# laclouis5/StructureDetector

Measured on AMD Instinct MI355X. Metric: images/sec (train fwd+bwd) and decode us/img at 512x512, higher is better.
Workload: dtype f32

## Files before the change

### include/sdnet_hip.h

```cpp
#ifndef SDNET_HIP_H
#define SDNET_HIP_H

#include <stddef.h>
#include <stdint.h>

#ifdef __cplusplus
extern "C" {
#endif

#define SD_ERR_INVALID   (-1)
#define SD_ERR_WORKSPACE (-2)
#define SD_ERR_ALIGN     (-3)

#define SD_MAX_TOPK 1024

typedef void* sd_stream_t;

int         sd_version(void);
const char* sd_last_error(void);
int         sd_build_flags(void);


int sd_clamped_sigmoid(const float* x, float* y, int64_t n, sd_stream_t stream);

// ... 218 lines not shown
int sd_conv2d_fwd_bf16(const void* x_nhwc_bf16, const void* w_krsc_bf16, void* y_nhwc_bf16, const sd_conv_desc* d,
                       const float* scale, const float* shift, const void* residual_bf16, int res_up2, int relu,
                       void* workspace, size_t workspace_bytes, sd_stream_t stream);
int sd_maxpool3x3s2_fwd_bf16(const void* x_bf16, void* y_bf16, int B, int Hi, int Wi, int C, sd_stream_t stream);
int sd_stem_bn_relu_maxpool_fwd_bf16(const float* x_nchw, const float* w, const float* scale, const float* shift, void* y_bf16,
                                     const sd_conv_desc* d, sd_stream_t stream);

int sd_cast_bf16_to_f32(const void* x_bf16, float* y, int64_t n, sd_stream_t stream);
size_t sd_conv2d_fwd_bf16_bn_stats_workspace_bytes(const sd_conv_desc* d);
int sd_conv2d_fwd_bf16_bn_stats(const void* x_nhwc_bf16, const void* w_krsc_bf16, void* y_nhwc_bf16, const sd_conv_desc* d, float eps,
                                float momentum, float* running_mean, float* running_var, float* mean, float* invstd,
                                void* workspace, size_t workspace_bytes, sd_stream_t stream);
int sd_conv2d_stem_fwd_bn_stats_bf16mm(const float* x_nchw, const float* w, float* y, const sd_conv_desc* d, float eps, float momentum,
                                       float* running_mean, float* running_var, float* mean, float* invstd,
                                       void* workspace, size_t workspace_bytes, sd_stream_t stream);
int sd_conv2d_stem_fwd_bn_stats_bf16(const float* x_nchw, const float* w, void* y_bf16, const sd_conv_desc* d, float eps, float momentum,
                                     float* running_mean, float* running_var, float* mean, float* invstd, void* workspace,
                                     size_t workspace_bytes, sd_stream_t stream);
int sd_bn_relu_maxpool_fwd_bf16(const void* x_bf16, int B, int Hi, int Wi, int C, const float* mean, const float* invstd, const float* gamma,
                                const float* beta, void* y_pool_bf16, uint8_t* idx, sd_stream_t stream);
int sd_maxpool_bn_relu_bwd_bf16(const void* dpool_bf16, const uint8_t* idx, const void* x_bf16, int B, int Hi, int Wi, int C, const float* mean,
                                const float* invstd, const float* gamma, const float* beta, float* dx, float* dgamma, float* dbeta, int accumulate,
                                void* workspace, size_t workspace_bytes, sd_stream_t stream);
int sd_maxpool_bn_relu_bwd_bf16_dx16(const void* dpool_bf16, const uint8_t* idx, const void* x_bf16, int B, int Hi, int Wi, int C, const float* mean,
                                     const float* invstd, const float* gamma, const float* beta, void* dx_bf16, float* dgamma, float* dbeta,
                                     int accumulate, void* workspace, size_t workspace_bytes, sd_stream_t stream);
int sd_conv2d_transpose_weights_bf16(const float* w, void* w_t_bf16, int Cout, int taps, int Cin, sd_stream_t stream);

int sd_conv2d_fwd_bf16_head_supported(const sd_conv_desc* d, int head_co);
size_t sd_head_split_bf16_bytes(void);
int sd_head_split_bf16(const float* head_w, const float* head_bias, int head_co, void* prepared, sd_stream_t stream);
int sd_conv2d_fwd_bf16_head(const void* x_bf16, const void* w_bf16, const sd_conv_desc* d, const float* scale, const float* shift, int relu,
                            const void* head_prepared, int head_co, float* head_y, sd_stream_t stream);
int sd_conv2d_dgrad_bf16(const void* dy_bf16, const void* w_t_bf16, void* dx_bf16, const sd_conv_desc* d, const void* residual_bf16,
                         int res_mode, sd_stream_t stream);
size_t sd_conv2d_wgrad_bf16_workspace_bytes(const sd_conv_desc* d);
int sd_conv2d_wgrad_bf16(const void* dy_bf16, const void* x_nhwc_bf16, float* dw_krsc, const sd_conv_desc* d, int accumulate,
                         void* workspace, size_t workspace_bytes, sd_stream_t stream);
int sd_bn_apply_bf16(const void* x, void* y, int64_t M, int C, const float* mean, const float* invstd, const float* gamma,
                     const float* beta, const void* residual, int relu, uint8_t* relu_mask_out, sd_stream_t stream);
int sd_bn_bwd_bf16(const void* dy, const void* x, const void* y, int relu, int64_t M, int C, const float* mean, const float* invstd,
                   const float* gamma, const float* beta, void* dx, void* g_out, float* dgamma, float* dbeta, int accumulate,
                   void* workspace, size_t workspace_bytes, sd_stream_t stream);
int sd_bn_train_stats_bf16(const void* x, int64_t M, int C, float eps, float momentum, float* running_mean, float* running_var,
                           float* mean, float* invstd, void* workspace, size_t workspace_bytes, sd_stream_t stream);
int sd_col_sum_bf16(const void* x, int64_t M, int C, float* out, int accumulate, void* workspace, size_t workspace_bytes, sd_stream_t stream);
int sd_upsample2x_bwd_bf16(const void* dy, const void* add, void* dx, int B, int H, int W, int C, sd_stream_t stream);
int sd_head_fwd_bf16(const void* x_nhwc_bf16, const float* w, const float* bias, float* y_nchw, int B, int HW, int C,
                     int Co, sd_stream_t stream);
int sd_conv2d_dgrad(const float* dy_nhwc, const float* w_t, float* dx_nhwc, const sd_conv_desc* d,
                    const float* residual, sd_stream_t stream);
int sd_conv2d_dgrad_half_res(const float* dy, const float* w_t, float* dx, const sd_conv_desc* d, const float* residual_half,
                             sd_stream_t stream);
int sd_conv2d_transpose_weights(const float* w, float* w_t, int Cout, int taps, int Cin, sd_stream_t stream);
int sd_conv2d_transpose_weights_batched(const float* w_base, void* w_t_base, const int* table, int nconv, int total_blocks, int out_bf16,
                                        sd_stream_t stream);
size_t sd_conv2d_wgrad_workspace_bytes(const sd_conv_desc* d);
int sd_conv2d_wgrad(const float* dy_nhwc, const float* x_nhwc, float* dw_krsc, const sd_conv_desc* d,
                    int accumulate, void* workspace, size_t workspace_bytes, sd_stream_t stream);
size_t sd_conv2d_stem_wgrad_workspace_bytes(const sd_conv_desc* d);
int sd_conv2d_stem_wgrad(const float* dy_nhwc, const float* x_nchw, float* dw_krsc, const sd_conv_desc* d,
                         int accumulate, void* workspace, size_t workspace_bytes, sd_stream_t stream);
int sd_conv2d_stem_wgrad_bf16mm(const float* dy, const float* x_nchw, float* dw, const sd_conv_desc* d, int accumulate, void* workspace,
                                size_t workspace_bytes, sd_stream_t stream);
int sd_conv2d_stem_wgrad_bf16(const void* dy_bf16, const float* x_nchw, float* dw, const sd_conv_desc* d, int accumulate, void* workspace,
                              size_t workspace_bytes, sd_stream_t stream);

size_t sd_col_reduce_workspace_bytes(int64_t M, int C);
int sd_bn_train_stats(const float* x, int64_t M, int C, float eps, float momentum, float* running_mean,
                      float* running_var, float* mean, float* invstd, void* workspace, size_t workspace_bytes,
                      sd_stream_t stream);
int sd_bn_apply(const float* x, float* y, int64_t M, int C, const float* mean, const float* invstd,
                const float* gamma, const float* beta, const float* residual, int relu, uint8_t* relu_mask_out,
                sd_stream_t stream);
int sd_bn_fold(const float* gamma, const float* beta, const float* running_mean, const float* running_var,
               float eps, int C, float* scale, float* shift, sd_stream_t stream);
int sd_bn_bwd(const float* dy, const float* x, const float* y, int relu, int64_t M, int C, const float* mean,
              const float* invstd, const float* gamma, const float* beta, float* dx, float* g_out, float* dgamma,
              float* dbeta, int accumulate, void* workspace, size_t workspace_bytes, sd_stream_t stream);
int sd_col_sum(const float* x, int64_t M, int C, float* out, int accumulate, void* workspace,
               size_t workspace_bytes, sd_stream_t stream);

int sd_maxpool3x3s2_fwd(const float* x, float* y, uint8_t* idx, int B, int Hi, int Wi, int C, sd_stream_t stream);
int sd_maxpool3x3s2_bwd(const float* dy, const uint8_t* idx, float* dx, int B, int Hi, int Wi, int C, sd_stream_t stream);
int sd_bn_relu_maxpool_fwd(const float* x, int B, int Hi, int Wi, int C, const float* mean, const float* invstd, const float* gamma,
                           const float* beta, float* y_pool, uint8_t* idx, sd_stream_t stream);
int sd_maxpool_bn_relu_bwd(const float* dpool, const uint8_t* idx, const float* x, int B, int Hi, int Wi, int C, const float* mean,
                           const float* invstd, const float* gamma, const float* beta, float* dx, float* dgamma, float* dbeta,
                           int accumulate, void* workspace, size_t workspace_bytes, sd_stream_t stream);
int sd_upsample2x_bwd(const float* dy, const float* add, float* dx, int B, int H, int W, int C, sd_stream_t stream);

#define SD_HEAD_MAX_CO 256
int sd_head_fwd(const float* x_nhwc, const float* w, const float* bias, float* y_nchw, int B, int HW, int C, int Co,
                sd_stream_t stream);
size_t sd_head_bwd_workspace_bytes(int B, int HW, int C, int Co);
int sd_head_bwd(const float* dy_nchw, const float* x_nhwc, const float* w, float* dx_nhwc, float* dw, float* dbias,
                int B, int HW, int C, int Co, int accumulate, void* workspace, size_t workspace_bytes, sd_stream_t stream);
int sd_head_bwd_bf16(const float* dy, const void* x_bf16, const float* w, void* dx_bf16, float* dw, float* dbias, int B, int HW, int C, int Co,
                     int accumulate, void* workspace, size_t workspace_bytes, sd_stream_t stream);

int sd_adam_step(float* param, const float* grad, float* exp_avg, float* exp_avg_sq, int64_t n, int step,
                 float lr, float beta1, float beta2, float eps, float grad_scale, sd_stream_t stream);

#define SD_OPTIM_STATUS_BYTES 16
size_t sd_grad_sumsq_workspace_bytes(int64_t n);
int sd_grad_sumsq(const float* grad, int64_t n, void* workspace, size_t workspace_bytes, sd_stream_t stream);
int sd_optim_step(float* param, const float* grad, float* exp_avg, float* exp_avg_sq, int64_t n, int step,
                  float lr, float beta1, float beta2, float eps, float grad_scale, float weight_decay,
                  const uint8_t* decay_mask, float max_norm, const void* partials, int npartials, float* ema,
                  float ema_decay, void* status, sd_stream_t stream);

#define SD_COMM_ID_BYTES 128
int sd_allreduce_unique_id(void* id_out);
int sd_allreduce_init(const void* id, int rank, int world, void** comm_out);
int sd_allreduce_run(void* comm, float* buf, int64_t count, sd_stream_t stream);
int sd_allreduce_destroy(void* comm);

int sd_comm_sim_copy(const void* src, void* dst, size_t src_bytes, size_t move_bytes, int workgroups, float gbps, sd_stream_t stream);

double sd_mfma_bf16_stream_flops(int iters);
int    sd_mfma_bf16_stream(const void* operands64k, float* out, int iters, sd_stream_t stream);

int sd_bn_stats_from_sums(const double* sums, int C, float eps, float momentum, float* running_mean, float* running_var, float* mean,
                          float* invstd, sd_stream_t stream);
int sd_bn_bwd_means_from_sums(const double* sums, int C, float* means_out, sd_stream_t stream);
int sd_bn_stats_sums(const float* partial, int rows, int64_t M, int C, double* sums, float* scratch, sd_stream_t stream);
int sd_bn_bwd_sums(const float* partial, int rows, int64_t M, int C, float* dgamma, float* dbeta, int accumulate, double* sums,
                   float* scratch, sd_stream_t stream);
int sd_bn_train_sums(const float* x, int64_t M, int C, double* sums, void* workspace, size_t workspace_bytes, sd_stream_t stream);
int sd_bn_train_sums_bf16(const void* x, int64_t M, int C, double* sums, void* workspace, size_t workspace_bytes, sd_stream_t stream);
int sd_conv2d_fwd_bn_stats_rows(const sd_conv_desc* d, int bf16);
int sd_conv2d_fwd_bn_sums(const float* x, const float* w, float* y, const sd_conv_desc* d, double* sums, void* workspace,
// ... 47 lines not shown
```

### structuredetector_amd/_lib.py

```python
from __future__ import annotations

import ctypes as C
import os
from pathlib import Path

import torch

_HERE = Path(__file__).resolve().parent
LIB_PATH = Path(os.environ.get("SDNET_HIP_LIB", _HERE / "csrc" / "libsdnet_hip.so"))

_lib = None

c_f32p = C.c_void_p
c_i64 = C.c_int64
c_int = C.c_int
c_float = C.c_float
c_size = C.c_size_t
c_vp = C.c_void_p


class SdError(RuntimeError):
    pass


# ... 64 lines not shown
    "sd_preprocess_images_list_jitter": (c_int, [c_vp] + [c_int] * 5 + [c_vp, c_vp, c_int, c_vp, c_vp, c_int, c_vp, c_vp, c_vp, C.POINTER(c_float),
                                                            C.POINTER(c_float), c_vp, c_vp, c_size, c_vp]),
    "sd_preprocess_affine_workspace_bytes": (c_size, [c_int] * 5),
    "sd_preprocess_images_affine": (c_int, [c_vp] + [c_int] * 5 + [c_vp, c_vp, c_int, c_vp, c_vp, c_int, c_vp, c_vp, c_vp, c_vp, C.POINTER(C.c_ubyte),
                                            C.POINTER(c_float), C.POINTER(c_float), c_vp, c_vp, c_size, c_vp]),
    "sd_preprocess_images_list_affine": (c_int, [c_vp] + [c_int] * 5 + [c_vp, c_vp, c_int, c_vp, c_vp, c_int, c_vp, c_vp, c_vp, c_vp, C.POINTER(C.c_ubyte),
                                                 C.POINTER(c_float), C.POINTER(c_float), c_vp, c_vp, c_size, c_vp]),
    "sd_preprocess_mosaic_workspace_bytes": (c_size, [c_int] * 5),
    "sd_preprocess_images_mosaic": (c_int, [c_vp] + [c_int] * 5 + [c_vp, c_vp, c_int, c_vp, c_vp, c_int, c_vp, c_vp, c_vp, c_vp, c_vp, c_vp,
                                            C.POINTER(C.c_ubyte), C.POINTER(c_float), C.POINTER(c_float), c_vp, c_vp, c_size, c_vp]),
    "sd_preprocess_images_list_mosaic": (c_int, [c_vp] + [c_int] * 5 + [c_vp, c_vp, c_int, c_vp, c_vp, c_int, c_vp, c_vp, c_vp, c_vp, c_vp, c_vp,
                                                 C.POINTER(C.c_ubyte), C.POINTER(c_float), C.POINTER(c_float), c_vp, c_vp, c_size, c_vp]),
    "sd_preprocess_window_workspace_bytes": (c_size, [c_int] * 4),
    "sd_preprocess_images_window": (c_int, [c_vp] + [c_int] * 7 + [c_vp, c_vp, c_int, c_vp, c_vp, c_int, c_vp, c_int, c_int] + [c_vp] * 6 +
                                    [C.POINTER(C.c_ubyte), C.POINTER(c_float), C.POINTER(c_float), c_vp, c_vp, c_size, c_vp]),
    "sd_preprocess_images_list_window": (c_int, [c_vp] + [c_int] * 7 + [c_vp, c_vp, c_int, c_vp, c_vp, c_int, c_vp, c_int, c_int] + [c_vp] * 6 +
                                         [C.POINTER(C.c_ubyte), C.POINTER(c_float), C.POINTER(c_float), c_vp, c_vp, c_size, c_vp]),
    "sd_render_targets": (c_int, [c_vp, c_vp, c_vp, c_int, c_int, c_int, c_int, c_float, c_vp, c_vp]),
    "sd_loss_workspace_bytes": (c_size, [c_int] * 5),
    "sd_loss_fwd": (c_int, [C.POINTER(LossDesc), c_vp, c_vp, c_size, c_vp]),
    "sd_loss_fwd_per_image": (c_int, [C.POINTER(LossDesc), c_vp, c_vp, c_size, c_vp]),
    "sd_loss_bwd": (c_int, [C.POINTER(LossDesc), c_vp, c_vp, c_vp, c_vp]),
    "sd_conv2d_fwd_workspace_bytes": (c_size, [C.POINTER(ConvDesc)]),
    "sd_conv2d_fwd": (c_int, [c_vp, c_vp, c_vp, C.POINTER(ConvDesc), c_vp, c_vp, c_vp, c_int, c_int, c_vp, c_size, c_vp]),
    "sd_conv2d_fwd_sb_supported": (c_int, [C.POINTER(ConvDesc), c_int]),
    "sd_conv2d_fwd_sb_workspace_bytes": (c_size, [C.POINTER(ConvDesc), c_int]),
    "sd_conv2d_fwd_sb_state_bytes": (c_size, [C.POINTER(ConvDesc), c_int]),
    "sd_conv2d_fwd_sb": (c_int, [c_vp, c_vp, c_vp, C.POINTER(ConvDesc), c_vp, c_vp, c_vp, c_int, c_int, c_int, c_vp, c_size, c_vp, c_size, c_vp]),
    "sd_conv2d_stem_fwd_workspace_bytes": (c_size, [C.POINTER(ConvDesc)]),
    "sd_conv2d_stem_fwd": (c_int, [c_vp, c_vp, c_vp, C.POINTER(ConvDesc), c_vp, c_vp, c_int, c_int, c_vp, c_size, c_vp]),
    "sd_cast_f32_to_bf16": (c_int, [c_vp, c_vp, c_i64, c_vp]),
    "sd_conv2d_fwd_bf16_workspace_bytes": (c_size, [C.POINTER(ConvDesc)]),
    "sd_conv2d_fwd_bf16": (c_int, [c_vp, c_vp, c_vp, C.POINTER(ConvDesc), c_vp, c_vp, c_vp, c_int, c_int, c_vp, c_size, c_vp]),
    "sd_conv2d_fwd_bf16_head_supported": (c_int, [C.POINTER(ConvDesc), c_int]),
    "sd_head_split_bf16_bytes": (c_size, []),
    "sd_head_split_bf16": (c_int, [c_vp, c_vp, c_int, c_vp, c_vp]),
    "sd_conv2d_fwd_bf16_head": (c_int, [c_vp, c_vp, C.POINTER(ConvDesc), c_vp, c_vp, c_int, c_vp, c_int, c_vp, c_vp]),
    "sd_cast_bf16_to_f32": (c_int, [c_vp, c_vp, c_i64, c_vp]),
    "sd_conv2d_fwd_bf16_bn_stats_workspace_bytes": (c_size, [c_vp]),
    "sd_conv2d_fwd_bf16_bn_stats": (c_int, [c_vp, c_vp, c_vp, c_vp, c_float, c_float, c_vp, c_vp, c_vp, c_vp, c_vp, c_size, c_vp]),
    "sd_conv2d_wgrad_bf16_workspace_bytes": (c_size, [c_vp]),
    "sd_conv2d_wgrad_bf16": (c_int, [c_vp, c_vp, c_vp, c_vp, c_int, c_vp, c_size, c_vp]),
    "sd_conv2d_transpose_weights_bf16": (c_int, [c_vp, c_vp, c_int, c_int, c_int, c_vp]),
    "sd_conv2d_dgrad_bf16": (c_int, [c_vp, c_vp, c_vp, c_vp, c_vp, c_int, c_vp]),
    "sd_bn_apply_bf16": (c_int, [c_vp, c_vp, c_i64, c_int, c_vp, c_vp, c_vp, c_vp, c_vp, c_int, c_vp, c_vp]),
    "sd_bn_bwd_bf16": (c_int, [c_vp, c_vp, c_vp, c_int, c_i64, c_int, c_vp, c_vp, c_vp, c_vp, c_vp, c_vp, c_vp, c_vp, c_int, c_vp, c_size, c_vp]),
    "sd_bn_train_stats_bf16": (c_int, [c_vp, c_i64, c_int, c_float, c_float, c_vp, c_vp, c_vp, c_vp, c_vp, c_size, c_vp]),
    "sd_col_sum_bf16": (c_int, [c_vp, c_i64, c_int, c_vp, c_int, c_vp, c_size, c_vp]),
    "sd_upsample2x_bwd_bf16": (c_int, [c_vp, c_vp, c_vp, c_int, c_int, c_int, c_int, c_vp]),
    "sd_maxpool3x3s2_fwd_bf16": (c_int, [c_vp, c_vp, c_int, c_int, c_int, c_int, c_vp]),
    "sd_stem_bn_relu_maxpool_fwd_bf16": (c_int, [c_vp, c_vp, c_vp, c_vp, c_vp, c_vp, c_vp]),
    "sd_head_fwd_bf16": (c_int, [c_vp, c_vp, c_vp, c_vp, c_int, c_int, c_int, c_int, c_vp]),
    "sd_conv2d_dgrad": (c_int, [c_vp, c_vp, c_vp, C.POINTER(ConvDesc), c_vp, c_vp]),
    "sd_conv2d_transpose_weights": (c_int, [c_vp, c_vp, c_int, c_int, c_int, c_vp]),
    "sd_conv2d_transpose_weights_batched": (c_int, [c_vp, c_vp, c_vp, c_int, c_int, c_int, c_vp]),
    "sd_conv2d_wgrad_workspace_bytes": (c_size, [C.POINTER(ConvDesc)]),
    "sd_conv2d_wgrad": (c_int, [c_vp, c_vp, c_vp, C.POINTER(ConvDesc), c_int, c_vp, c_size, c_vp]),
    "sd_conv2d_stem_wgrad_workspace_bytes": (c_size, [C.POINTER(ConvDesc)]),
    "sd_conv2d_stem_wgrad": (c_int, [c_vp, c_vp, c_vp, C.POINTER(ConvDesc), c_int, c_vp, c_size, c_vp]),
    "sd_conv2d_stem_wgrad_bf16mm": (c_int, [c_vp, c_vp, c_vp, C.POINTER(ConvDesc), c_int, c_vp, c_size, c_vp]),
    "sd_conv2d_stem_wgrad_bf16": (c_int, [c_vp, c_vp, c_vp, C.POINTER(ConvDesc), c_int, c_vp, c_size, c_vp]),
    "sd_col_reduce_workspace_bytes": (c_size, [c_i64, c_int]),
    "sd_bn_train_stats": (c_int, [c_vp, c_i64, c_int, c_float, c_float, c_vp, c_vp, c_vp, c_vp, c_vp, c_size, c_vp]),
    "sd_bn_apply": (c_int, [c_vp, c_vp, c_i64, c_int, c_vp, c_vp, c_vp, c_vp, c_vp, c_int, c_vp, c_vp]),
    "sd_bn_fold": (c_int, [c_vp, c_vp, c_vp, c_vp, c_float, c_int, c_vp, c_vp, c_vp]),
    "sd_bn_bwd": (c_int, [c_vp, c_vp, c_vp, c_int, c_i64, c_int, c_vp, c_vp, c_vp, c_vp, c_vp, c_vp, c_vp, c_vp, c_int, c_vp, c_size, c_vp]),
    "sd_col_sum": (c_int, [c_vp, c_i64, c_int, c_vp, c_int, c_vp, c_size, c_vp]),
    "sd_maxpool3x3s2_fwd": (c_int, [c_vp, c_vp, c_vp, c_int, c_int, c_int, c_int, c_vp]),
    "sd_maxpool3x3s2_bwd": (c_int, [c_vp, c_vp, c_vp, c_int, c_int, c_int, c_int, c_vp]),
    "sd_upsample2x_bwd": (c_int, [c_vp, c_vp, c_vp, c_int, c_int, c_int, c_int, c_vp]),
    "sd_head_fwd": (c_int, [c_vp, c_vp, c_vp, c_vp, c_int, c_int, c_int, c_int, c_vp]),
    "sd_head_bwd_workspace_bytes": (c_size, [c_int] * 4),
    "sd_head_bwd": (c_int, [c_vp] * 6 + [c_int] * 5 + [c_vp, c_size, c_vp]),
    "sd_head_bwd_bf16": (c_int, [c_vp] * 6 + [c_int] * 5 + [c_vp, c_size, c_vp]),
    "sd_adam_step": (c_int, [c_vp, c_vp, c_vp, c_vp, c_i64, c_int, c_float, c_float, c_float, c_float, c_float, c_vp]),
    "sd_grad_sumsq_workspace_bytes": (c_size, [c_i64]),
    "sd_grad_sumsq": (c_int, [c_vp, c_i64, c_vp, c_size, c_vp]),
    "sd_optim_step": (c_int, [c_vp, c_vp, c_vp, c_vp, c_i64, c_int, c_float, c_float, c_float, c_float, c_float, c_float, c_vp, c_float, c_vp, c_int,
                              c_vp, c_float, c_vp, c_vp]),
    "sd_conv2d_kernel_name": (C.c_char_p, [c_vp, c_int]),
    "sd_set_option": (c_int, [C.c_char_p, c_int]),
    "sd_decode_set_option": (c_int, [C.c_char_p, c_int]),
    "sd_decode_kernel_names": (C.c_char_p, [c_int] * 9),
    "sd_conv2d_stem_fwd_bn_stats_workspace_bytes": (c_size, [c_vp]),
    "sd_conv2d_stem_fwd_bn_stats": (c_int, [c_vp, c_vp, c_vp, c_vp, c_float, c_float, c_vp, c_vp, c_vp, c_vp, c_vp, c_size, c_vp]),
    "sd_conv2d_stem_fwd_bn_stats_bf16mm": (c_int, [c_vp, c_vp, c_vp, c_vp, c_float, c_float, c_vp, c_vp, c_vp, c_vp, c_vp, c_size, c_vp]),
    "sd_conv2d_stem_fwd_bn_stats_bf16": (c_int, [c_vp, c_vp, c_vp, c_vp, c_float, c_float, c_vp, c_vp, c_vp, c_vp, c_vp, c_size, c_vp]),
    "sd_conv2d_dgrad_half_res": (c_int, [c_vp] * 6),
    "sd_bn_relu_maxpool_fwd": (c_int, [c_vp, c_int, c_int, c_int, c_int] + [c_vp] * 7),
    "sd_bn_relu_maxpool_fwd_bf16": (c_int, [c_vp, c_int, c_int, c_int, c_int] + [c_vp] * 7),
    "sd_maxpool_bn_relu_bwd": (c_int, [c_vp, c_vp, c_vp, c_int, c_int, c_int, c_int] + [c_vp] * 7 + [c_int, c_vp, c_size, c_vp]),
    "sd_maxpool_bn_relu_bwd_bf16": (c_int, [c_vp, c_vp, c_vp, c_int, c_int, c_int, c_int] + [c_vp] * 7 + [c_int, c_vp, c_size, c_vp]),
    "sd_maxpool_bn_relu_bwd_bf16_dx16": (c_int, [c_vp, c_vp, c_vp, c_int, c_int, c_int, c_int] + [c_vp] * 7 + [c_int, c_vp, c_size, c_vp]),
    "sd_conv2d_fwd_bn_stats_workspace_bytes": (c_size, [c_vp]),
    "sd_conv2d_fwd_bn_stats": (c_int, [c_vp, c_vp, c_vp, c_vp, c_float, c_float, c_vp, c_vp, c_vp, c_vp, c_vp, c_size, c_vp]),
    "sd_conv2d_dgrad_bn_reduce_workspace_bytes": (c_size, [c_vp]),
    "sd_conv2d_dgrad_bn_reduce": (c_int, [c_vp] * 5 + [c_vp, c_vp, c_int] + [c_vp] * 6 + [c_int, c_vp, c_vp, c_size, c_vp]),
    "sd_bn_bwd_finalize": (c_int, [c_vp, c_int, c_i64, c_int, c_vp, c_vp, c_int, c_vp, c_vp, c_vp]),
    "sd_bn_bwd_apply": (c_int, [c_vp, c_vp, c_vp, c_int, c_i64, c_int] + [c_vp] * 8),
    "sd_bn_finalize_scratch_rows": (c_int, [c_int]),
    "sd_bn_finalize_stats": (c_int, [c_vp, c_int, c_i64, c_int, c_float, c_float, c_vp, c_vp, c_vp, c_vp, c_vp, c_vp]),
    "sd_bn_stats_from_sums": (c_int, [c_vp, c_int, c_float, c_float, c_vp, c_vp, c_vp, c_vp, c_vp]),
    "sd_bn_bwd_means_from_sums": (c_int, [c_vp, c_int, c_vp, c_vp]),
    "sd_bn_stats_sums": (c_int, [c_vp, c_int, c_i64, c_int, c_vp, c_vp, c_vp]),
    "sd_bn_bwd_sums": (c_int, [c_vp, c_int, c_i64, c_int, c_vp, c_vp, c_int, c_vp, c_vp, c_vp]),
    "sd_bn_train_sums": (c_int, [c_vp, c_i64, c_int, c_vp, c_vp, c_size, c_vp]),
# ... 114 lines not shown
```

### structuredetector_amd/csrc/sd_conv.hip

```cpp
#include <string.h>
#include "sd_common.h"
#include "sd_mfma.h"
#include "sd_conv_rows.h"

#ifndef SD_S2_LPT
#define SD_S2_LPT 1
#endif
namespace sd {


#ifndef SD_IGEMM_DMA
#define SD_IGEMM_DMA 1
#endif
#ifndef SD_ABLATE_HOT
#define SD_ABLATE_HOT 0
#endif
#ifndef SD_ABLATE_STORE
#define SD_ABLATE_STORE 0
#endif
#ifndef SD_ABLATE_PATCH
#define SD_ABLATE_PATCH 0
#endif
#if SD_ABLATE_HOT || SD_ABLATE_STORE || SD_ABLATE_PATCH || defined(SD_PP_ABL) || defined(SD_RS_ABL)
#warning "timing-only ablation build: this libsdnet_hip.so computes WRONG RESULTS; the Python loader refuses it unless SDNET_ALLOW_ABLATION=1"
// ... 10 lines not shown
#if defined(SD_PP_ABL) || defined(SD_RS_ABL) || defined(SD_SB_ABL) || defined(SD_SHAPE_EXP) || defined(SD_W16_ABL) || defined(SD_SR_ABL) || defined(SD_SF_ABL)
#define SD_EXPERIMENT_FLAG 16
#else
#define SD_EXPERIMENT_FLAG 0
#endif
void sd_nn_set_pool_pair(int v);
extern "C" int sd_build_flags(void) { return (SD_ABLATE_HOT ? 1 : 0) | (SD_ABLATE_STORE ? 2 : 0) | (SD_ABLATE_PATCH ? 4 : 0) | SD_TRACE_FLAG | SD_EXPERIMENT_FLAG; }

#ifndef SD_SHAPE_EXP
#define SD_SHAPE_EXP 0
#else
#define SD_SHAPE_EXP_BUILD 1
#endif
__device__ __forceinline__ f32x16 mfma_shape_exp(bf16x8 a, bf16x8 b, f32x16 c) {
    f32x4 c0 = __builtin_shufflevector(c, c, 0, 1, 2, 3), c1 = __builtin_shufflevector(c, c, 4, 5, 6, 7);
    c0 = __builtin_amdgcn_mfma_f32_16x16x32_bf16(a, b, c0, 0, 0, 0);
    c1 = __builtin_amdgcn_mfma_f32_16x16x32_bf16(b, a, c1, 0, 0, 0);
    c[0] = c0[0]; c[1] = c0[1]; c[2] = c0[2]; c[3] = c0[3]; c[4] = c1[0]; c[5] = c1[1]; c[6] = c1[2]; c[7] = c1[3];
    return c;
}
#define SD_MFMA_BF16(BIT, a, b, c) (((SD_SHAPE_EXP) & (BIT)) ? mfma_shape_exp(a, b, c) : __builtin_amdgcn_mfma_f32_32x32x16_bf16(a, b, c, 0, 0, 0))

#ifndef SD_IGEMM_LATE_DMA
#define SD_IGEMM_LATE_DMA 0
#endif
constexpr int NBUF = 2;
constexpr int BM = 128, BK = 32, LDK = BK;

struct ConvArgs {
    const void* x;
    const void* w;
    void* y;
    const float* scale;
    const float* shift;
    const void* res;
    int B, Hi, Wi, Ck, Ho, Wo, Nn, R, S;
    int mul, div, off, rsign;
    int relu, res_up2;
    int M, nk, kchunks;
    int splits;
    float* part;
    const float* bn_x;
    const float* bn_y;
    const float *bn_mean, *bn_invstd, *bn_gamma, *bn_beta;
    int bn_relu;
    float* stat;
    int pt_tw_log2, pt_pw, pt_pieces, pt_rolling, pt_flip;
    int pt_strip_log2;
    int par;
    const uint16_t* head_w;
    const float* head_b;
    float* head_y;
    int head_co;
};

__device__ __attribute__((aligned(128))) float g_zero_line[64];


__device__ __forceinline__ void s2_tile(int bid, int nwg, int n_tiles, int off, int& cls, int& tq, int& n_idx, int& tile_m) {
    if (SD_S2_LPT && (nwg & 31) == 0) {
        const int xcd = bid & 7, pos = bid >> 3, per = nwg >> 5;
        const int k4 = pos / per, within = xcd * per + (pos - k4 * per);
        cls = (off & 1) ? (k4 == 0 ? 3 : k4 == 3 ? 0 : k4) : k4;
        tq = within / n_tiles; n_idx = within - tq * n_tiles;
    } else {
        const int tile = xcd_remap(bid, nwg), tm = tile / n_tiles;
        cls = tm & 3; tq = tm >> 2; n_idx = tile - tm * n_tiles;
    }
    tile_m = 4 * tq + cls;
}


__device__ __forceinline__ float f4c(const float4& v, int t) { return t == 0 ? v.x : (t == 1 ? v.y : (t == 2 ? v.z : v.w)); }

struct BnRed4 { float4 mu, is, ga, be, s, q; };
__device__ __forceinline__ void bnred4_init(BnRed4& b, const ConvArgs& p, int n) {
    b.mu = *reinterpret_cast<const float4*>(p.bn_mean + n); b.is = *reinterpret_cast<const float4*>(p.bn_invstd + n);
    b.ga = b.be = b.s = b.q = make_float4(0.f, 0.f, 0.f, 0.f);
    if (p.bn_relu == 2) { b.ga = *reinterpret_cast<const float4*>(p.bn_gamma + n); b.be = *reinterpret_cast<const float4*>(p.bn_beta + n); }
}
__device__ __forceinline__ void bnred4_add(BnRed4& b, const ConvArgs& p, float4 g, int64_t m, int n) {
    const int64_t i = m * p.Nn + n;
    const float4 xv = *reinterpret_cast<const float4*>(p.bn_x + i);
    const float4 xh = make_float4((xv.x - b.mu.x) * b.is.x, (xv.y - b.mu.y) * b.is.y, (xv.z - b.mu.z) * b.is.z, (xv.w - b.mu.w) * b.is.w);
    if (p.bn_relu == 1) {
        const float4 yy = *reinterpret_cast<const float4*>(p.bn_y + i);
        g.x = yy.x > 0.f ? g.x : 0.f; g.y = yy.y > 0.f ? g.y : 0.f; g.z = yy.z > 0.f ? g.z : 0.f; g.w = yy.w > 0.f ? g.w : 0.f;
    } else if (p.bn_relu == 3) {
        const uint8_t mb = reinterpret_cast<const uint8_t*>(p.bn_y)[i >> 2];
        g.x = (mb & 1) ? g.x : 0.f; g.y = (mb & 2) ? g.y : 0.f; g.z = (mb & 4) ? g.z : 0.f; g.w = (mb & 8) ? g.w : 0.f;
    } else if (p.bn_relu == 2) {
        g.x = (xh.x * b.ga.x + b.be.x) > 0.f ? g.x : 0.f; g.y = (xh.y * b.ga.y + b.be.y) > 0.f ? g.y : 0.f;
        g.z = (xh.z * b.ga.z + b.be.z) > 0.f ? g.z : 0.f; g.w = (xh.w * b.ga.w + b.be.w) > 0.f ? g.w : 0.f;
    }
    b.s.x += g.x; b.s.y += g.y; b.s.z += g.z; b.s.w += g.w;
    b.q.x += g.x * xh.x; b.q.y += g.y * xh.y; b.q.z += g.z * xh.z; b.q.w += g.w * xh.w;
}
template <int LPR>
__device__ __forceinline__ void bnred4_wave_sum(BnRed4& b) {
#pragma unroll
    for (int o = LPR; o < 64; o <<= 1) {
        b.s.x += __shfl_xor(b.s.x, o); b.s.y += __shfl_xor(b.s.y, o); b.s.z += __shfl_xor(b.s.z, o); b.s.w += __shfl_xor(b.s.w, o);
        b.q.x += __shfl_xor(b.q.x, o); b.q.y += __shfl_xor(b.q.y, o); b.q.z += __shfl_xor(b.q.z, o); b.q.w += __shfl_xor(b.q.w, o);
    }
}

// ... 380 lines not shown
            if (BF16) {
                uint2 pk;
                pk.x = (uint32_t)f2bf(v.x) | ((uint32_t)f2bf(v.y) << 16);
                pk.y = (uint32_t)f2bf(v.z) | ((uint32_t)f2bf(v.w) << 16);
                *reinterpret_cast<uint2*>(reinterpret_cast<uint16_t*>(p.y) + (int64_t)m * p.Nn + n) = pk;
            } else {
                *reinterpret_cast<float4*>(reinterpret_cast<float*>(p.y) + (int64_t)m * p.Nn + n) = v;
                if (bwd_red) bnred4_add(br, p, v, m, n);
            }
        };
        if constexpr (BF16) {
#pragma unroll
            for (int it = 0; it < 64 / RPI; ++it) out_row(it, rr[it], nullptr);
        } else if (pre32) {
#pragma unroll
            for (int it = 0; it < 64 / RPI; ++it) out_row(it, make_uint2(0u, 0u), &rf[it]);
        } else {
#pragma unroll 4
            for (int it = 0; it < 64 / RPI; ++it) out_row(it, make_uint2(0u, 0u), nullptr);
        }
        if (bwd_red) {
            bnred4_wave_sum<LPR>(br);
            if ((wave >> 1) == 1 && lane < LPR) {
                *reinterpret_cast<float4*>(&statred[0][wn0 + c4]) = br.s; *reinterpret_cast<float4*>(&statred[1][wn0 + c4]) = br.q;
            }
            __syncthreads();
            if ((wave >> 1) == 0 && lane < LPR) {
                float* dst = p.stat + (int64_t)tile_m * 2 * p.Nn + n;
                const float4 a = *reinterpret_cast<const float4*>(&statred[0][wn0 + c4]), bq = *reinterpret_cast<const float4*>(&statred[1][wn0 + c4]);
                *reinterpret_cast<float4*>(dst) = make_float4(br.s.x + a.x, br.s.y + a.y, br.s.z + a.z, br.s.w + a.w);
                *reinterpret_cast<float4*>(dst + p.Nn) = make_float4(br.q.x + bq.x, br.q.y + bq.y, br.q.z + bq.z, br.q.w + bq.w);
            }
            red_done = true;
        }
    }
    if (fwd_stat || (bwd_red && !red_done)) {
#pragma unroll
        for (int ni = 0; ni < NT; ++ni) {
            sv[ni] += __shfl_xor(sv[ni], 32); qv[ni] += __shfl_xor(qv[ni], 32);
            if ((wave >> 1) == 1 && fh == 0) { statred[0][wn0 + ni * 32 + fr] = sv[ni]; statred[1][wn0 + ni * 32 + fr] = qv[ni]; }
        }
        __syncthreads();
        if ((wave >> 1) == 0 && fh == 0) {
            float* dst = p.stat + (int64_t)tile_m * 2 * p.Nn + n0;
#pragma unroll
            for (int ni = 0; ni < NT; ++ni) {
                const int c = wn0 + ni * 32 + fr;
                dst[c] = sv[ni] + statred[0][c]; dst[p.Nn + c] = qv[ni] + statred[1][c];
            }
        }
    }
}

template <int BN, int WM, int WN, int MT, int NTW, bool FWD, bool BF16 = false, bool VEC = false, typename RowMap, typename ResMap>
__device__ __forceinline__ void tile_epilogue(const ConvArgs& p, f32x16 (&acc)[MT][NTW], RowMap row_to_m, ResMap row_to_res, int tid, int wave, int fr,
                                              int fh, int wm0, int wn0, int n0, int tile_m, float* T0 = nullptr, float* T1 = nullptr) {
    const bool fwd_stat = FWD && p.stat && !p.bn_x;
    const bool bwd_red = !BF16 && p.stat && p.bn_x;
    float sv[NTW], qv[NTW];
#pragma unroll
    for (int ni = 0; ni < NTW; ++ni) {
        sv[ni] = qv[ni] = 0.f;
        if (fwd_stat) {
#pragma unroll
            for (int mi = 0; mi < MT; ++mi)
#pragma unroll
                for (int e = 0; e < 16; ++e) { const float a = BF16 ? bf2f(f2bf(acc[mi][ni][e])) : acc[mi][ni][e]; sv[ni] += a; qv[ni] += a * a; }
        }
    }
    const int lane = tid & 63;
    bool red_done = false;
    __shared__ float statred[2][BN];
    if (VEC && NTW == 2) {
        const int c4 = (lane & 15) * 4, n = n0 + wn0 + c4;
        float4 sc4 = make_float4(1.f, 1.f, 1.f, 1.f), sh4 = make_float4(0.f, 0.f, 0.f, 0.f);
        if (p.scale) sc4 = *reinterpret_cast<const float4*>(p.scale + n);
        if (p.shift) sh4 = *reinterpret_cast<const float4*>(p.shift + n);
        BnRed4 br;
        if (bwd_red) bnred4_init(br, p, n);
        const bool two = T1 != nullptr;
        const int npass = two ? MT / 2 : MT, rpp = two ? 64 : 32;
        for (int h = 0; h < npass; ++h) {
            uint2 rr[16] = {};
            if constexpr (BF16) {
                if (p.res) {
#pragma unroll
                    for (int it = 0; it < 16; ++it) {
                        if (it * 4 < rpp) {
                            const int trow = wm0 + h * rpp + it * 4 + (lane >> 4);
                            const int m = row_to_m(trow);
                            const int64_t rm = m < 0 ? -1 : (p.res_up2 ? (int64_t)row_to_res(trow, m) : (int64_t)m);
                            rr[it] = *reinterpret_cast<const uint2*>(reinterpret_cast<const uint16_t*>(p.res) + (rm >= 0 ? rm * p.Nn : 0) + n);
                        }
                    }
                }
            }
#pragma unroll
            for (int ni = 0; ni < NTW; ++ni)
#pragma unroll
                for (int e = 0; e < 16; ++e) {
                    const int r = (e & 3) + 8 * (e >> 2) + 4 * fh;
                    float v0 = 0.f, v1 = 0.f;
#pragma unroll
                    for (int mi = 0; mi < MT; ++mi) {
                        if (two ? mi == 2 * h : mi == h) v0 = acc[mi][ni][e];
                        if (two && mi == 2 * h + 1) v1 = acc[mi][ni][e];
                    }
                    T0[r * 64 + ni * 32 + fr] = v0;
                    if (two) T1[r * 64 + ni * 32 + fr] = v1;
                }
            auto out_row = [&](int it, uint2 r16) {
                const int rl = it * 4 + (lane >> 4);
                const int trow = wm0 + h * rpp + rl;
                const int m = row_to_m(trow);
                if (m < 0) return;
                float4 v = *reinterpret_cast<const float4*>((rl < 32 ? T0 : T1) + (rl & 31) * 64 + c4);
                v.x = v.x * sc4.x + sh4.x; v.y = v.y * sc4.y + sh4.y; v.z = v.z * sc4.z + sh4.z; v.w = v.w * sc4.w + sh4.w;
                if (p.res) {
                    const int64_t rm = p.res_up2 ? (int64_t)row_to_res(trow, m) : (int64_t)m;
                    if (rm >= 0) {
                        if (BF16) {
                            v.x += bf2f((uint16_t)(r16.x & 0xffff)); v.y += bf2f((uint16_t)(r16.x >> 16));
                            v.z += bf2f((uint16_t)(r16.y & 0xffff)); v.w += bf2f((uint16_t)(r16.y >> 16));
                        } else {
                            const float4 r = *reinterpret_cast<const float4*>(reinterpret_cast<const float*>(p.res) + rm * p.Nn + n);
                            v.x += r.x; v.y += r.y; v.z += r.z; v.w += r.w;
                        }
                    }
                }
                if (p.relu) { v.x = fmaxf(v.x, 0.f); v.y = fmaxf(v.y, 0.f); v.z = fmaxf(v.z, 0.f); v.w = fmaxf(v.w, 0.f); }
                if (BF16) {
                    uint2 pk;
                    pk.x = (uint32_t)f2bf(v.x) | ((uint32_t)f2bf(v.y) << 16);
                    pk.y = (uint32_t)f2bf(v.z) | ((uint32_t)f2bf(v.w) << 16);
                    *reinterpret_cast<uint2*>(reinterpret_cast<uint16_t*>(p.y) + (int64_t)m * p.Nn + n) = pk;
                } else {
                    *reinterpret_cast<float4*>(reinterpret_cast<float*>(p.y) + (int64_t)m * p.Nn + n) = v;
                    if (bwd_red) bnred4_add(br, p, v, m, n);
                }
            };
            if constexpr (BF16) {
#pragma unroll
                for (int it = 0; it < 16; ++it)
                    if (it * 4 < rpp) out_row(it, rr[it]);
            } else {
#pragma unroll 4
                for (int it = 0; it < 16; ++it) {
                    if (it * 4 >= rpp) break;
                    out_row(it, make_uint2(0u, 0u));
                }
            }
        }
        if (bwd_red) {
            bnred4_wave_sum<16>(br);
            if (tid < 2 * BN) statred[tid / BN][tid % BN] = 0.f;
            __syncthreads();
            for (int wr = 1; wr < WM; ++wr) {
                if (wave / WN == wr && lane < 16) {
                    float4* a = reinterpret_cast<float4*>(&statred[0][wn0 + c4]);
                    float4* bq = reinterpret_cast<float4*>(&statred[1][wn0 + c4]);
                    *a = make_float4(a->x + br.s.x, a->y + br.s.y, a->z + br.s.z, a->w + br.s.w);
                    *bq = make_float4(bq->x + br.q.x, bq->y + br.q.y, bq->z + br.q.z, bq->w + br.q.w);
                }
                __syncthreads();
            }
            if (wave / WN == 0 && lane < 16) {
                float* dst = p.stat + (int64_t)tile_m * 2 * p.Nn + n;
                const float4 a = *reinterpret_cast<const float4*>(&statred[0][wn0 + c4]), bq = *reinterpret_cast<const float4*>(&statred[1][wn0 + c4]);
                *reinterpret_cast<float4*>(dst) = make_float4(br.s.x + a.x, br.s.y + a.y, br.s.z + a.z, br.s.w + a.w);
                *reinterpret_cast<float4*>(dst + p.Nn) = make_float4(br.q.x + bq.x, br.q.y + bq.y, br.q.z + bq.z, br.q.w + bq.w);
            }
            red_done = true;
        }
    } else {
#pragma unroll
    for (int ni = 0; ni < NTW; ++ni) {
        const int n = n0 + wn0 + ni * 32 + fr;
        const float sc = p.scale ? p.scale[n] : 1.f;
        const float sh = p.shift ? p.shift[n] : 0.f;
        float bmu = 0.f, bis = 0.f, bga = 0.f, bbe = 0.f;
        if (bwd_red) {
            bmu = p.bn_mean[n]; bis = p.bn_invstd[n];
            if (p.bn_relu == 2) { bga = p.bn_gamma[n]; bbe = p.bn_beta[n]; }
        }
#pragma unroll
        for (int mi = 0; mi < MT; ++mi) {
#pragma unroll
            for (int e = 0; e < 16; ++e) {
                const int trow = wm0 + mi * 32 + (e & 3) + 8 * (e >> 2) + 4 * fh;
                const int m = row_to_m(trow);
                if (m < 0) continue;
                float v = acc[mi][ni][e] * sc + sh;
                if (p.res) {
                    const int64_t rm = p.res_up2 ? row_to_res(trow, m) : m;
                    const bool has = rm >= 0;
                    if (has) v += BF16 ? bf2f(reinterpret_cast<const uint16_t*>(p.res)[rm * p.Nn + n]) : reinterpret_cast<const float*>(p.res)[rm * p.Nn + n];
                }
                if (p.relu) v = fmaxf(v, 0.f);
                if (BF16) reinterpret_cast<uint16_t*>(p.y)[(int64_t)m * p.Nn + n] = f2bf(v);
                else if (!SD_ABLATE_STORE || v == 123.456f) reinterpret_cast<float*>(p.y)[(int64_t)m * p.Nn + n] = v;
                if (bwd_red) SD_BNRED_TERM(v, m, n, sv[ni], qv[ni])
            }
        }
// ... 393 lines not shown
        f32x4 a00 = lds_read128_async<0>(aa[0]), a01 = lds_read128_async<0>(aa[1]);                \
        f32x4 a02 = a00, a03 = a00;                                                                \
        if (MT == 4) { a02 = lds_read128_async<0>(aa[MT - 2]); a03 = lds_read128_async<0>(aa[MT - 1]); } \
        f32x4 b00 = lds_read128_async<0>(bb), b01 = lds_read128_async<TSTR>(bb);                   \
        f32x4 a10 = lds_read128_async<0>(aa[0] ^ 32u), a11 = lds_read128_async<0>(aa[1] ^ 32u);    \
        f32x4 a12 = a10, a13 = a10;                                                                \
        if (MT == 4) { a12 = lds_read128_async<0>(aa[MT - 2] ^ 32u); a13 = lds_read128_async<0>(aa[MT - 1] ^ 32u); } \
        f32x4 b10 = lds_read128_async<0>(bb ^ 32u), b11 = lds_read128_async<TSTR>(bb ^ 32u);       \
         \
        if (BF16 || SD_PATCH_READS_FIRST_F32) {                                                    \
            PT_ISSUE_B(cc + ((t) + 2) / 9, ((t) + 2) % 9, ((t) + 2) % 3)                               \
        if (rolling) {                                                                             \
             \
            if ((t) < 8) {                                                                         \
                const int row = (t) < 4 ? 2 + (t) / 2 : ((t) - 4) / 2;                             \
                const int cch = (t) < 4 ? cc : cc + 1;                                             \
                if (cch < nchunks) {                                                               \
                    if (((t) & 1) == 0) { PT_PATCH(3 * row, Pt, cch * KC) ++n_iss; }               \
                    else {                                                                         \
                        if (PT_OWN(3 * row + 1)) { PT_PATCH(3 * row + 1, Pt, cch * KC) ++n_iss; }  \
                        if (PT_OWN(3 * row + 2)) { PT_PATCH(3 * row + 2, Pt, cch * KC) ++n_iss; }  \
                    }                                                                              \
                }                                                                                  \
            }                                                                                      \
        } else if ((t) < 7 && cc + 1 < nchunks && PT_OWN(t)) {                                     \
            PT_PATCH(t, pt_nxt, (cc + 1) * KC) ++n_iss;                                            \
        }                                                                                          \
        }                                                                                          \
        if (MT == 4) { SD_LDS_WAIT6(6, a00, a01, a02, a03, b00, b01); } else { SD_LDS_WAIT4(4, a00, a01, b00, b01); } \
        PT_MFMA_GROUP(a00, a01, a02, a03, b00, b01)                                                \
        if (MT == 4) { SD_LDS_WAIT6(0, a10, a11, a12, a13, b10, b11); } else { SD_LDS_WAIT4(0, a10, a11, b10, b11); } \
        PT_MFMA_GROUP(a10, a11, a12, a13, b10, b11)                                                \
         \
        if (n_iss == PBW) wait_vmcnt_and_lds<PBW>();                                               \
        else if (n_iss == PBW + 1) wait_vmcnt_and_lds<PBW + 1>();                                  \
        else wait_vmcnt_and_lds<PBW + 2>();                                                        \
        __builtin_amdgcn_s_barrier();                                                              \
    }
    for (int cc = 0; cc < nchunks; ++cc) {
        const uint32_t pt_cur = pt_base + (rolling ? 0u : (uint32_t)(cc & 1) * (PT_STAGE_FLOATS * 4));
        float* const pt_nxt = Pt + (rolling ? 0 : ((cc + 1) & 1) * PT_STAGE_FLOATS);
        PT_TAP(0) PT_TAP(1) PT_TAP(2) PT_TAP(3) PT_TAP(4) PT_TAP(5) PT_TAP(6) PT_TAP(7) PT_TAP(8)
    }
    wait_vmcnt<0>();
#undef PT_TAP
#undef PT_MFMA_GROUP
#undef PT_MFMA1
#undef PT_ISSUE_B
#undef PT_OWN
#undef PT_PATCH
#undef PT_PB
    __syncthreads();
    float* T0 = BN == 128 ? (wave < 3 ? Pt + wave * 4096 : Bs) : Pt + wave * 2048;
    tile_epilogue<BN, WM, WN, MT, NTW, true, BF16, true>(
        p, acc, [&](int row) { return m0 + row; },
        [&](int, int m) {
            const int ox = m % p.Wo, t = m / p.Wo, oy = t % p.Ho, b = t / p.Ho;
            return (p.res_up2 == 2 && ((ox | oy) & 1)) ? -1 : (b * (p.Ho >> 1) + (oy >> 1)) * (p.Wo >> 1) + (ox >> 1);
        },
        tid, wave, fr, fh, wm0, wn0, n0, tile_m, T0, BN == 128 ? T0 + 2048 : nullptr);
}

template <int BN, bool BF16 = false>
__global__ __launch_bounds__(256, 2) void k_conv3x3_patch(ConvArgs p) { conv3x3_patch_body<BN, BF16, false>(p); }
template <int BN, bool BF16 = false>
__global__ __launch_bounds__(256, 2) void k_conv3x3_patch_roll(ConvArgs p) { conv3x3_patch_body<BN, BF16, true>(p); }

typedef float pp_f32x2 __attribute__((ext_vector_type(2)));
template <bool HEAD>
__device__ __forceinline__ void pp_epilogue_bf16(const ConvArgs& p, f32x4 (&acc)[4][8], int mbase, int TWl, int tid, int wave, int n0, int tile_m,
                                                 float* T0, float* T1) {
    constexpr int BN = 128;
    const int lane = tid & 63, r16 = lane & 15, kq = lane >> 4;
    const int wml = (wave & 3) * 64;
    const bool fwd_stat = p.stat && !p.bn_x;
    float sv[8], qv[8];
#pragma unroll
    for (int ni = 0; ni < 8; ++ni) {
        sv[ni] = qv[ni] = 0.f;
        if (fwd_stat) {
#pragma unroll
            for (int mi = 0; mi < 4; ++mi)
#pragma unroll
                for (int e = 0; e < 4; ++e) { const float a = bf2f(f2bf(acc[mi][ni][e])); sv[ni] += a; qv[ni] += a * a; }
        }
    }
    __shared__ float pp_statred[2][BN];
    const int c4 = (lane & 15) * 4;
    const bool affine = p.scale || p.shift;
    const int TWm = (1 << TWl) - 1, rsub = lane >> 4;
    f32x4 hacc[4][2];
    if constexpr (HEAD) {
#pragma unroll
        for (int mi = 0; mi < 4; ++mi) { hacc[mi][0] = f32x4{0.f, 0.f, 0.f, 0.f}; hacc[mi][1] = f32x4{0.f, 0.f, 0.f, 0.f}; }
    }
    const bool head2 = HEAD && p.head_co > 16;
#pragma unroll
    for (int h = 0; h < 2; ++h) {
        const int n = n0 + h * 64 + c4;
        bf16x8 hw[2][2][2];
        if constexpr (HEAD) {
#pragma unroll
            for (int ks = 0; ks < 2; ++ks)
#pragma unroll
                for (int no = 0; no < 2; ++no)
#pragma unroll
                    for (int hl = 0; hl < 2; ++hl)
// ... 625 lines not shown
#undef RS_MFMA2
            asm volatile("s_nop 15\n\ts_nop 15" ::: "memory");
#undef RS_ADDR
#undef RS_SCR_RD
            if (p.res) {
#pragma unroll
                for (int it = 0; it < 4; ++it) resv[it] = resn[it];
            }
            PP_T(r3_)
            wait_vmcnt<0>();
            PP_T(r4_)
#pragma unroll
            for (int ni = 0; ni < 2; ++ni)
#pragma unroll
                for (int e = 0; e < 16; ++e)
                    scr[((e & 3) + 8 * (e >> 2) + 4 * fh) * RS_SCR + ni * 32 + fr] = acc[ni][e] * sc[ni] + sh[ni];
            PP_T(r5_)
            __syncthreads();
            PP_T(r6_)
            PP_ACC(2, r0_, r3_) PP_ACC(3, r3_, r4_) PP_ACC(4, r4_, r5_) PP_ACC(5, r5_, r6_)
#ifdef SD_PP_TRACE
            tr[7] += 1;
#endif
        }
#ifdef SD_PP_TRACE
        if (blockIdx.x == 8 && lane == 0) { for (int k = 0; k < 8; ++k) g_pp_trace[wave][k] = tr[k]; }
#endif
        store_row(y1 - 1);
        if (p.stat) {
#pragma unroll
            for (int k = 0; k < 8; ++k) {
                float a = ssum[k], q = ssq[k];
                for (int o = 8; o < 64; o <<= 1) { a += __shfl_xor(a, o); q += __shfl_xor(q, o); }
                if (lane < 8) { sred[wave * 128 + lane * 8 + k] = a; sred[wave * 128 + 64 + lane * 8 + k] = q; }
            }
            __syncthreads();
            if (tid < 128) p.stat[(int64_t)unit * 128 + tid] = (sred[tid] + sred[128 + tid]) + (sred[256 + tid] + sred[384 + tid]);
        }
        wait_vmcnt<0>();
        __syncthreads();
    }
}

constexpr int RF_PX = 72, RF_ROW_BYTES = RF_PX * 256, RF_NR = 5, RF_B_AGPR = 240;
constexpr int RF_LDS_BYTES = RF_NR * RF_ROW_BYTES + 4 * 64 * 4;

struct RowsArgsF {
    const float* x;
    const float* w;
    float* y;
    const float* scale;
    const float* shift;
    const float* res;
    float* stat;
    int relu, flip;
    int B, H, W, segs, rows, units_per_col, nunits;
};

template <bool B_IN_AGPR, bool ZERO>
__device__ __forceinline__ void rf_mfma(f32x16& acc, float a, float b) {
#if defined(__HIP_DEVICE_COMPILE__)
    if constexpr (ZERO) {
        if constexpr (B_IN_AGPR) asm volatile("v_mfma_f32_32x32x2_f32 %0, %1, %2, 0" : "=a"(acc) : "v"(a), "a"(b));
        else asm volatile("v_mfma_f32_32x32x2_f32 %0, %1, %2, 0" : "=a"(acc) : "v"(a), "v"(b));
    } else {
        if constexpr (B_IN_AGPR) asm volatile("v_mfma_f32_32x32x2_f32 %0, %1, %2, %0" : "+a"(acc) : "v"(a), "a"(b));
        else asm volatile("v_mfma_f32_32x32x2_f32 %0, %1, %2, %0" : "+a"(acc) : "v"(a), "v"(b));
    }
#else
    (void)acc; (void)a; (void)b;
#endif
}

__global__ __launch_bounds__(256) void k_conv3x3_c64_rows_f32(RowsArgsF p) {
    extern __shared__ __attribute__((aligned(16))) float rf_lds[];
    char* const ring = reinterpret_cast<char*>(rf_lds);
    const int tid = threadIdx.x, lane = tid & 63, wave = __builtin_amdgcn_readfirstlane(tid >> 6);
    const int ph = wave & 1, chh = wave >> 1;
    float* const sred = reinterpret_cast<float*>(ring + RF_NR * RF_ROW_BYTES);
    const int fr = lane & 31, fh = lane >> 5;
    const float* const zero_ = g_zero_line;

    float Bw[288];
#pragma unroll
    for (int t = 0; t < 9; ++t)
#pragma unroll
        for (int q = 0; q < 8; ++q) {
            const float4 v = *reinterpret_cast<const float4*>(p.w + ((chh * 32 + fr) * 9 + (p.flip ? 8 - t : t)) * 64 + 8 * q + 4 * fh);
            Bw[t * 32 + 4 * q + 0] = v.x; Bw[t * 32 + 4 * q + 1] = v.y; Bw[t * 32 + 4 * q + 2] = v.z; Bw[t * 32 + 4 * q + 3] = v.w;
        }
    const float sc = p.scale ? p.scale[chh * 32 + fr] : 1.f, sh = p.shift ? p.shift[chh * 32 + fr] : 0.f;
    uint32_t aoff[3][4];
#pragma unroll
    for (int s3 = 0; s3 < 3; ++s3) {
        const int pxr = ph * 32 + fr + s3;
#pragma unroll
        for (int qq = 0; qq < 4; ++qq) aoff[s3][qq] = (uint32_t)pxr * 256u + ((uint32_t)((2 * qq + fh) ^ (pxr & 7)) << 4);
    }
    const int dpx = lane >> 4, dslot = lane & 15;

    for (int unit = blockIdx.x; unit < p.nunits; unit += gridDim.x) {
        const int col = unit / p.units_per_col, yu = unit - col * p.units_per_col;
        const int b = col / p.segs, x0 = (col - b * p.segs) * 64;
        const int y0 = yu * p.rows, y1 = min(y0 + p.rows, p.H);
        const float* const img = p.x + (int64_t)b * p.H * p.W * 64;
        auto issue_row = [&](int iy) {
            float* const dst = reinterpret_cast<float*>(ring + ((iy - y0 + 1) % RF_NR) * RF_ROW_BYTES);
#pragma unroll
            for (int j = 0; j < 5; ++j) {
                const int pc = wave + 4 * j;
                if (pc < 18) {
                    const int pxr = pc * 4 + dpx, ix = x0 - 1 + pxr;
                    const bool ok = pxr < 66 && (unsigned)ix < (unsigned)p.W && (unsigned)iy < (unsigned)p.H;
                    lds_dma16(ok ? img + ((int64_t)iy * p.W + ix) * 64 + ((dslot ^ (pxr & 7)) << 2) : zero_ + (dslot << 2), dst + pc * 256);
                }
            }
        };
        float ssum = 0.f, ssq = 0.f;
        for (int iy = y0 - 1; iy <= min(y0 + 2, y1); ++iy) issue_row(iy);
        wait_vmcnt<0>();
        __syncthreads();
        const uint32_t ring_base = lds_addr(ring);
#ifdef SD_PP_TRACE
        unsigned long long tr[8] = {0, 0, 0, 0, 0, 0, 0, 0};
#endif
        for (int y = y0; y < y1; ++y) {
            PP_T(r0_)
            float resv[16];
            const int64_t orow = (((int64_t)b * p.H + y) * p.W + x0 + ph * 32 + 4 * fh) * 64 + chh * 32 + fr;
            if (p.res) {
#pragma unroll
                for (int e = 0; e < 16; ++e) resv[e] = p.res[orow + ((e & 3) + 8 * (e >> 2)) * 64];
            }
            const bool more = y + 3 <= y1;
            float* const ddst = reinterpret_cast<float*>(ring + ((y + 3 - y0 + 1) % RF_NR) * RF_ROW_BYTES);
            const float* dsrc[5];
#pragma unroll
            for (int j = 0; j < 5; ++j) {
                const int pxr = (wave + 4 * j) * 4 + dpx, ix = x0 - 1 + pxr;
                const bool ok = pxr < 66 && (unsigned)ix < (unsigned)p.W && (unsigned)(y + 3) < (unsigned)p.H;
                dsrc[j] = ok ? img + ((int64_t)(y + 3) * p.W + ix) * 64 + ((dslot ^ (pxr & 7)) << 2) : zero_ + (dslot << 2);
                asm volatile("" : "+v"(dsrc[j]));
            }
            uint32_t ad[3][3][4];
#pragma unroll
            for (int r = 0; r < 3; ++r) {
                const uint32_t sb = ring_base + (uint32_t)((y - 1 + r - y0 + 1) % RF_NR) * RF_ROW_BYTES;
#pragma unroll
                for (int s3 = 0; s3 < 3; ++s3)
#pragma unroll
                    for (int qq = 0; qq < 4; ++qq) ad[r][s3][qq] = sb + aoff[s3][qq];
            }
            f32x16 acc;
#define RF_RD(i) lds_read128_async<(((i) % 8) >> 2) * 128>(ad[((i) / 8) / 3][((i) / 8) % 3][(i) % 4])
            f32x4 A[4];
            PP_T(r1_)
            A[0] = RF_RD(0); A[1] = RF_RD(1); A[2] = RF_RD(2);
#define RF_STEP(i)                                                                                                     \
            {                                                                                                          \
                if ((i) + 3 < 72) A[((i) + 3) & 3] = RF_RD((i) + 3 < 72 ? (i) + 3 : 0);                                   \
                                              \
                if ((i) + 3 < 72) asm volatile("s_waitcnt lgkmcnt(3)" : "+v"(A[(i) & 3]) :: "memory");                   \
                else if ((i) == 69) asm volatile("s_waitcnt lgkmcnt(2)" : "+v"(A[(i) & 3]) :: "memory");                 \
                else if ((i) == 70) asm volatile("s_waitcnt lgkmcnt(1)" : "+v"(A[(i) & 3]) :: "memory");                 \
                else asm volatile("s_waitcnt lgkmcnt(0)" : "+v"(A[(i) & 3]) :: "memory");                                \
                if ((i) < 5 && more && wave + 4 * (i) < 18) lds_dma16(dsrc[(i) < 5 ? (i) : 0], ddst + (wave + 4 * (i)) * 256);  \
                const f32x4 a_ = A[(i) & 3];                                                                           \
                rf_mfma<(4 * (i) + 0 < RF_B_AGPR), (i) == 0>(acc, a_[0], Bw[4 * (i) + 0]);                              \
                rf_mfma<(4 * (i) + 1 < RF_B_AGPR), false>(acc, a_[1], Bw[4 * (i) + 1]);                                 \
                rf_mfma<(4 * (i) + 2 < RF_B_AGPR), false>(acc, a_[2], Bw[4 * (i) + 2]);                                 \
                rf_mfma<(4 * (i) + 3 < RF_B_AGPR), false>(acc, a_[3], Bw[4 * (i) + 3]);                                 \
                __builtin_amdgcn_sched_barrier(0);                                                                     \
            }
#define RF_TAP(t) RF_STEP(8 * (t)) RF_STEP(8 * (t) + 1) RF_STEP(8 * (t) + 2) RF_STEP(8 * (t) + 3) RF_STEP(8 * (t) + 4) RF_STEP(8 * (t) + 5) RF_STEP(8 * (t) + 6) RF_STEP(8 * (t) + 7)
            RF_TAP(0) RF_TAP(1) RF_TAP(2) RF_TAP(3) RF_TAP(4) RF_TAP(5) RF_TAP(6) RF_TAP(7) RF_TAP(8)
#undef RF_TAP
#undef RF_STEP
#undef RF_RD
            asm volatile("s_nop 15\n\ts_nop 15" ::: "memory");
            PP_T(r2_)
            wait_vmcnt<0>();
            PP_T(r3_)
#pragma unroll
            for (int e = 0; e < 16; ++e) {
                float v = acc[e] * sc + sh;
                if (p.res) v += resv[e];
                if (p.relu) v = fmaxf(v, 0.f);
                ssum += v; ssq += v * v;
                p.y[orow + ((e & 3) + 8 * (e >> 2)) * 64] = v;
            }
            PP_T(r4_)
            __builtin_amdgcn_s_barrier();
            PP_T(r5_)
            PP_ACC(0, r0_, r1_) PP_ACC(1, r1_, r2_) PP_ACC(2, r2_, r3_) PP_ACC(3, r3_, r4_) PP_ACC(4, r4_, r5_)
#ifdef SD_PP_TRACE
            tr[7] += 1;
#endif
        }
#ifdef SD_PP_TRACE
        if (blockIdx.x == 8 && lane == 0) { for (int kk = 0; kk < 8; ++kk) g_pp_trace[wave][kk] = tr[kk]; }
#endif
        if (p.stat) {
            ssum += __shfl_xor(ssum, 32); ssq += __shfl_xor(ssq, 32);
            if (fh == 0) { sred[wave * 64 + fr] = ssum; sred[wave * 64 + 32 + fr] = ssq; }
            __syncthreads();
            if (tid < 128) {
                const int which = tid >> 6, n = tid & 63, cw = (n >> 5) * 2;
                p.stat[(int64_t)unit * 128 + tid] = sred[cw * 64 + which * 32 + (n & 31)] + sred[(cw + 1) * 64 + which * 32 + (n & 31)];
            }
        }
        __syncthreads();
    }
}

#undef SD_BNRED_TERM

struct WgradArgs {
    const float* dy;
    const float* x;
    float* part;
    int B, Hi, Wi, Ck, Ho, Wo, Nn, R, S, stride, pad;
    int M, splits, m_per_split;
    int strips, chunks_total, chunks_per_split;
};

template <int TN, int TC>
__global__ __launch_bounds__(256, 2) void k_conv_wgrad(WgradArgs p) {
    constexpr int PK = 32;
    constexpr int LDN = TN + 4, LDC = TC + 4;
    constexpr int NT = TN / 64, CT = TC / 64;
    constexpr int DV = PK * TN / 4 / 256, XV = PK * TC / 4 / 256;
    extern __shared__ __attribute__((aligned(16))) float lds[];
    float* Ds = lds;
    float* Xs = lds + 2 * PK * LDN;

// ... 2391 lines not shown
    a.pt_tw_log2 = l2;
    a.pt_rolling = a.Wo == 128;
    a.pt_pw = a.pt_rolling ? 144 : a.Wo + 2;
    a.pt_pieces = a.pt_rolling ? 36 : cdiv((th + 2) * a.pt_pw, 16);
    a.pt_flip = a.rsign < 0;
    return a.pt_pieces * 256 <= (a.pt_rolling ? PT_FLOATS : PT_STAGE_FLOATS);
}

static thread_local int g_patch_narrow = 2;
static int patch_tile_bn(ConvArgs& a, int BN, int mode, bool bf16) {
    ConvArgs t = a;
    if (conv_patch_geometry(t, BN, mode, bf16, false, g_patch_min_tiles)) { a = t; return BN; }
    if (BN == 128 && (bf16 ? g_patch_narrow >= 2 : g_patch_narrow >= 1)) {
        t = a;
        if (conv_patch_geometry(t, 64, mode, bf16, true, g_patch_min_tiles)) { a = t; return 64; }
    }
    return 0;
}

static thread_local int g_rows64_min_units = 192;
static bool conv_rows64_geometry(const ConvArgs& a, int mode, RowsArgs& r) {
    if (mode != 0 || a.Ck != 64 || a.Nn != 64 || a.R != 3 || a.S != 3 || a.mul != 1 || a.div != 1 || a.splits > 1) return false;
    if (!((a.rsign == 1 && a.off == -1) || (a.rsign == -1 && a.off == 1))) return false;
    if (a.Ho != a.Hi || a.Wo != a.Wi || a.Wo % 128 || a.res_up2 || a.bn_x) return false;
    r = RowsArgs{};
    r.B = a.B; r.H = a.Ho; r.W = a.Wo; r.segs = a.Wo / 128;
    const int cols = r.B * r.segs;
    r.rows = std::min(r.H, std::max(8, cdiv(r.H * cols, 256)));
    r.units_per_col = cdiv(r.H, r.rows);
    r.nunits = cols * r.units_per_col;
    if (r.nunits < g_rows64_min_units || (g_rows64_min_units > 1 && r.rows < 16)) return false;
    r.x = (const uint16_t*)a.x; r.w = (const uint16_t*)a.w; r.y = (uint16_t*)a.y; r.scale = a.scale; r.shift = a.shift;
    r.res = (const uint16_t*)a.res; r.stat = a.stat; r.relu = a.relu; r.flip = a.rsign < 0;
    return true;
}

static thread_local int g_rows16 = 1;
static bool conv_rows16_args(const RowsArgs& r) { return g_rows16 && !r.stat; }

static thread_local int g_rowsf32_min_units = 192;
static thread_local int g_stem_fwd_blocks = 512;
static bool conv_rowsf32_geometry(const ConvArgs& a, int mode, RowsArgsF& r) {
    if (mode != 0 || a.Ck != 64 || a.Nn != 64 || a.R != 3 || a.S != 3 || a.mul != 1 || a.div != 1 || a.splits > 1) return false;
    if (!((a.rsign == 1 && a.off == -1) || (a.rsign == -1 && a.off == 1))) return false;
    if (a.Ho != a.Hi || a.Wo != a.Wi || a.Wo % 64 || a.res_up2 || a.bn_x) return false;
    r = RowsArgsF{};
    r.B = a.B; r.H = a.Ho; r.W = a.Wo; r.segs = a.Wo / 64;
    const int cols = r.B * r.segs;
    r.rows = std::min(r.H, std::max(8, cdiv(r.H * cols, 256)));
    r.units_per_col = cdiv(r.H, r.rows);
    r.nunits = cols * r.units_per_col;
    if (r.nunits < g_rowsf32_min_units || (g_rowsf32_min_units > 1 && r.rows < 16)) return false;
    r.x = (const float*)a.x; r.w = (const float*)a.w; r.y = (float*)a.y; r.scale = a.scale; r.shift = a.shift;
    r.res = (const float*)a.res; r.stat = a.stat; r.relu = a.relu; r.flip = a.rsign < 0;
    return true;
}

static thread_local int g_pp_min_tiles = 200;
static thread_local int g_pp_strips = 1;
static bool conv_pp_geometry(ConvArgs& a, int mode, int min_tiles) {
    if (a.Nn % 128 || a.M % PP_BM || (a.M / PP_BM) * (a.Nn / 128) < min_tiles || a.res_up2) return false;
    a.pt_strip_log2 = 0;
    int l2 = 0;
    while ((1 << l2) < a.Wo) ++l2;
    if (g_pp_strips && (1 << l2) == a.Wo && a.Wo >= 128 && a.Wo <= 4096 && a.Ho % 4 == 0) {
        if (!SD_CONV_PATCH || mode != 0 || a.R != 3 || a.S != 3 || a.mul != 1 || a.div != 1 || a.splits > 1) return false;
        if (!((a.rsign == 1 && a.off == -1) || (a.rsign == -1 && a.off == 1))) return false;
        if (a.Ho != a.Hi || a.Wo != a.Wi || a.Ck % 32) return false;
        a.pt_tw_log2 = 6; a.pt_strip_log2 = l2 - 6; a.pt_rolling = 0; a.pt_pw = 66; a.pt_pieces = cdiv(6 * 66, 16); a.pt_flip = a.rsign < 0;
        return true;
    }
    return conv_patch_geometry(a, 128, mode, true, false, 1) && !a.pt_rolling;
}

static thread_local int g_stem_fwd_ring = 1;
static thread_local int g_igemm_big_bf16 = 0;
static int igemm_big_tiles(const ConvArgs& a, int BN, int mode) {
    if (!SD_IGEMM_BIG || (BN != 128 && !SD_IGEMM_BIG64 && !(SD_IGEMM_BIG64_S2 && mode == 2)) || (mode != 0 && mode != 2) || a.splits > 1) return 0;
    if (a.R * a.S * a.Ck < 512) return 0;
    const int m_per = mode == 2 ? a.M / 4 : a.M;
    const int big_tiles = (mode == 2 ? 4 : 1) * cdiv(m_per, BMB) * (a.Nn / BN);
    return (big_tiles >= 512 && (mode != 2 || m_per % BMB == 0)) ? big_tiles : 0;
}

enum ConvFamily {
    CONV_STREAM1X1,
    CONV_ROWS16,
    CONV_ROWS_BF16,
    CONV_ROWS_F32,
    CONV_PP,
    CONV_PP_HEAD,
    CONV_PATCH,
    CONV_PATCH_ROLL,
    CONV_IGEMM_BIG,
    CONV_IGEMM,
};

struct ConvPlan {
    ConvFamily family;
    bool bf16;
    int BN, mode;
    int grid_x, grid_y, block;
    size_t lds;
    int stat_rows;
    ConvArgs a;
    RowsArgs ra;
    RowsArgsF rf;
// ... 553 lines not shown
}

int sd_conv2d_stem_fwd_bn_stats_bf16(const float* x_nchw, const float* w, void* y_bf16, const sd_conv_desc* d, float eps, float momentum,
                                     float* running_mean, float* running_var, float* mean, float* invstd, void* workspace,
                                     size_t workspace_bytes, sd_stream_t stream) {
    return stem_fwd_bn_stats_bf16("sd_conv2d_stem_fwd_bn_stats_bf16", x_nchw, w, y_bf16, d, eps, momentum, running_mean, running_var, mean, invstd,
                                  nullptr, workspace, workspace_bytes, stream);
}

int sd_conv2d_stem_fwd_bn_sums(const float* x_nchw, const float* w, float* y, const sd_conv_desc* d, double* sums, void* workspace,
                               size_t workspace_bytes, sd_stream_t stream) {
    SD_REQUIRE(sums, SD_ERR_INVALID, "sd_conv2d_stem_fwd_bn_sums: null pointer");
    return stem_fwd_bn_stats_f32("sd_conv2d_stem_fwd_bn_sums", x_nchw, w, y, d, 0.f, 0.f, nullptr, nullptr, nullptr, nullptr, sums, workspace,
                                 workspace_bytes, stream);
}

int sd_conv2d_stem_fwd_bn_sums_bf16mm(const float* x_nchw, const float* w, float* y, const sd_conv_desc* d, double* sums, void* workspace,
                                      size_t workspace_bytes, sd_stream_t stream) {
    SD_REQUIRE(sums, SD_ERR_INVALID, "sd_conv2d_stem_fwd_bn_sums_bf16mm: null pointer");
    return stem_fwd_bn_stats_bf16mm("sd_conv2d_stem_fwd_bn_sums_bf16mm", x_nchw, w, y, d, 0.f, 0.f, nullptr, nullptr, nullptr, nullptr, sums,
                                    workspace, workspace_bytes, stream);
}

int sd_conv2d_stem_fwd_bn_sums_bf16(const float* x_nchw, const float* w, void* y_bf16, const sd_conv_desc* d, double* sums, void* workspace,
                                    size_t workspace_bytes, sd_stream_t stream) {
    SD_REQUIRE(sums, SD_ERR_INVALID, "sd_conv2d_stem_fwd_bn_sums_bf16: null pointer");
    return stem_fwd_bn_stats_bf16("sd_conv2d_stem_fwd_bn_sums_bf16", x_nchw, w, y_bf16, d, 0.f, 0.f, nullptr, nullptr, nullptr, nullptr, sums,
                                  workspace, workspace_bytes, stream);
}

int sd_conv2d_dgrad_half_res(const float* dy, const float* w_t, float* dx, const sd_conv_desc* d, const float* residual_half,
                             sd_stream_t stream) {
    if (int e = check_conv("sd_conv2d_dgrad_half_res", d)) return e;
    SD_REQUIRE(dy && w_t && dx && residual_half, SD_ERR_INVALID, "sd_conv2d_dgrad_half_res: null pointer");
    SD_REQUIRE(d->Cout % 32 == 0 && d->Cin % 64 == 0, SD_ERR_INVALID, "sd_conv2d_dgrad_half_res: needs Cout %% 32 == 0 and Cin %% 64 == 0");
    SD_REQUIRE(d->Hi % 2 == 0 && d->Wi % 2 == 0, SD_ERR_INVALID, "sd_conv2d_dgrad_half_res: needs even Hi, Wi");
    SD_REQUIRE(aligned16(dy) && aligned16(w_t) && aligned16(dx) && aligned16(residual_half), SD_ERR_ALIGN,
               "sd_conv2d_dgrad_half_res: pointers must be 16-byte aligned");
    ConvArgs a = conv_args(d, 1, false);
    a.x = dy; a.w = w_t; a.y = dx; a.res = residual_half; a.res_up2 = 2;
    return launch_igemm(a, false, (hipStream_t)stream);
}

int sd_conv2d_dgrad(const float* dy, const float* w_t, float* dx, const sd_conv_desc* d, const float* residual, sd_stream_t stream) {
    if (int e = check_conv("sd_conv2d_dgrad", d)) return e;
    SD_REQUIRE(dy && w_t && dx, SD_ERR_INVALID, "sd_conv2d_dgrad: null pointer");
    SD_REQUIRE(d->Cout % 32 == 0 && d->Cin % 64 == 0, SD_ERR_INVALID, "sd_conv2d_dgrad: needs Cout %% 32 == 0 and Cin %% 64 == 0");
    SD_REQUIRE(aligned16(dy) && aligned16(w_t) && aligned16(dx) && aligned16(residual), SD_ERR_ALIGN, "sd_conv2d_dgrad: pointers must be 16-byte aligned");
    ConvArgs a = conv_args(d, 1, false);
    a.x = dy; a.w = w_t; a.y = dx; a.res = residual;
    return launch_igemm(a, false, (hipStream_t)stream);
}

int sd_conv2d_transpose_weights(const float* w, float* w_t, int Cout, int taps, int Cin, sd_stream_t stream) {
    SD_REQUIRE(w && w_t && Cout > 0 && taps > 0 && Cin > 0, SD_ERR_INVALID, "sd_conv2d_transpose_weights: bad arguments");
    hipLaunchKernelGGL(k_transpose_w<float>, dim3(cdiv(Cin, 32), cdiv(Cout, 32), taps), dim3(256), 0, (hipStream_t)stream, w, w_t, Cout, taps, Cin);
    SD_LAUNCH_CHECK();
    return 0;
}

int sd_conv2d_transpose_weights_bf16(const float* w, void* w_t_bf16, int Cout, int taps, int Cin, sd_stream_t stream) {
    SD_REQUIRE(w && w_t_bf16 && Cout > 0 && taps > 0 && Cin > 0, SD_ERR_INVALID, "sd_conv2d_transpose_weights_bf16: bad arguments");
    hipLaunchKernelGGL(k_transpose_w<uint16_t>, dim3(cdiv(Cin, 32), cdiv(Cout, 32), taps), dim3(256), 0, (hipStream_t)stream, w, (uint16_t*)w_t_bf16,
                       Cout, taps, Cin);
    SD_LAUNCH_CHECK();
    return 0;
}

int sd_conv2d_transpose_weights_batched(const float* w_base, void* w_t_base, const int* table, int nconv, int total_blocks, int out_bf16,
                                        sd_stream_t stream) {
    SD_REQUIRE(w_base && w_t_base && table && nconv > 0 && total_blocks > 0, SD_ERR_INVALID, "sd_conv2d_transpose_weights_batched: bad arguments");
    if (out_bf16) hipLaunchKernelGGL(k_transpose_w_batched<uint16_t>, dim3(total_blocks), dim3(256), 0, (hipStream_t)stream, w_base, (uint16_t*)w_t_base, table, nconv);
    else hipLaunchKernelGGL(k_transpose_w_batched<float>, dim3(total_blocks), dim3(256), 0, (hipStream_t)stream, w_base, (float*)w_t_base, table, nconv);
    SD_LAUNCH_CHECK();
    return 0;
}

static bool wgrad_all_taps(const sd_conv_desc* d) {
    return d->Cin % 64 == 0 && d->Cout % 64 == 0 && d->R == 3 && d->S == 3 && d->stride == 1 && d->pad == 1 &&
           (d->Wo % 32 == 0 || (d->Wo == 16 && d->Ho % 2 == 0));
}

static thread_local int g_wgrad_f32_ring = 2;
static thread_local int g_wgrad_bf16_ring = 5;
static int wgrad_tile_splits(const sd_conv_desc* d, int tiles) {
    const int M = d->B * d->Ho * d->Wo;
    const bool small = (d->Cout % 128 != 0) && (d->Cin % 128 != 0);
    const int slots = 256 * (small ? 4 : 2);
    const int max_s = std::max(1, cdiv(M, 512));
    int best_s = 1;
    double best_fill = 0.0;
    for (int k = 1; k <= 4; ++k) {
        int s = std::min(std::max(1, k * slots / tiles), max_s);
        const int rounds = cdiv(tiles * s, slots);
        const double fill = (double)tiles * s / ((double)rounds * slots);
        if (fill > best_fill + 0.03) { best_fill = fill; best_s = s; }
    }
    return best_s;
}

enum WgradFamily {
    WGRAD_TAPS_RING2,
    WGRAD_TAPS_RING,
    WGRAD_TAPS,
    WGRAD_TILE,
    WGRAD_TAP_BF16,
// ... 371 lines not shown
```

### structuredetector_amd/csrc/sd_nn.hip

```cpp
#include "sd_common.h"
#include "sd_mfma.h"
#include <type_traits>

namespace sd {

constexpr int RED_ROWS_PER_BLOCK = 256;

template <int MODE, typename T = float>
__global__ __launch_bounds__(256) void k_col_reduce(const T* __restrict__ a, const T* __restrict__ b, const T* __restrict__ y,
                                                     const float* __restrict__ mean, const float* __restrict__ invstd,
                                                     const float* __restrict__ gamma, const float* __restrict__ beta, int relu,
                                                     int64_t M, int C, float* __restrict__ partial, int rpb) {
    __shared__ float4 red[2][256];
    const int cols = C >> 2;
    const int lanes = 256 / cols;
    const int col = threadIdx.x % cols, rl = threadIdx.x / cols;
    const int64_t r0 = (int64_t)blockIdx.x * rpb;
    const int64_t r1 = min(r0 + rpb, M);
    float4 s0 = make_float4(0.f, 0.f, 0.f, 0.f), s1 = s0;
    float4 mu = s0, is = s0, ga = s0, be = s0;
    if (MODE == 1 && rl < lanes) {
        mu = reinterpret_cast<const float4*>(mean)[col];
        is = reinterpret_cast<const float4*>(invstd)[col];
        if (relu == 2) { ga = reinterpret_cast<const float4*>(gamma)[col]; be = reinterpret_cast<const float4*>(beta)[col]; }
    }
    if (rl < lanes) {
#pragma unroll 4
        for (int64_t r = r0 + rl; r < r1; r += lanes) {
            const float4 v = ld4(a, r * cols + col);
            if (MODE == 0) {
                s0.x += v.x; s0.y += v.y; s0.z += v.z; s0.w += v.w;
                s1.x += v.x * v.x; s1.y += v.y * v.y; s1.z += v.z * v.z; s1.w += v.w * v.w;
            } else if (MODE == 2) {
                s0.x += v.x; s0.y += v.y; s0.z += v.z; s0.w += v.w;
            } else {
                float4 g = v;
                const float4 xv = ld4(b, r * cols + col);
                if (relu == 1) {
                    const float4 yy = ld4(y, r * cols + col);
                    g.x = yy.x > 0.f ? g.x : 0.f; g.y = yy.y > 0.f ? g.y : 0.f;
                    g.z = yy.z > 0.f ? g.z : 0.f; g.w = yy.w > 0.f ? g.w : 0.f;
                } else if (relu == 2) {
                    g.x = ((xv.x - mu.x) * is.x * ga.x + be.x) > 0.f ? g.x : 0.f; g.y = ((xv.y - mu.y) * is.y * ga.y + be.y) > 0.f ? g.y : 0.f;
                    g.z = ((xv.z - mu.z) * is.z * ga.z + be.z) > 0.f ? g.z : 0.f; g.w = ((xv.w - mu.w) * is.w * ga.w + be.w) > 0.f ? g.w : 0.f;
                } else if (relu == 3) {
                    const uint8_t mb = reinterpret_cast<const uint8_t*>(y)[r * cols + col];
                    g.x = (mb & 1) ? g.x : 0.f; g.y = (mb & 2) ? g.y : 0.f; g.z = (mb & 4) ? g.z : 0.f; g.w = (mb & 8) ? g.w : 0.f;
                }
                s0.x += g.x; s0.y += g.y; s0.z += g.z; s0.w += g.w;
                s1.x += g.x * ((xv.x - mu.x) * is.x); s1.y += g.y * ((xv.y - mu.y) * is.y);
                s1.z += g.z * ((xv.z - mu.z) * is.z); s1.w += g.w * ((xv.w - mu.w) * is.w);
            }
        }
    }
    red[0][threadIdx.x] = s0;
    red[1][threadIdx.x] = s1;
    __syncthreads();
    if (rl == 0) {
        for (int l = 1; l < lanes; ++l) {
            const float4 u = red[0][l * cols + col], w = red[1][l * cols + col];
            s0.x += u.x; s0.y += u.y; s0.z += u.z; s0.w += u.w;
            s1.x += w.x; s1.y += w.y; s1.z += w.z; s1.w += w.w;
        }
        float* dst = partial + (int64_t)blockIdx.x * 2 * C;
        reinterpret_cast<float4*>(dst)[col] = s0;
        reinterpret_cast<float4*>(dst + C)[col] = s1;
    }
}

__global__ __launch_bounds__(256) void k_rows_fold(const float* __restrict__ in, int rows, int W, int slab, float* __restrict__ out) {
    __shared__ float4 red[256];
    const int cols = W >> 2, lanes = 256 / cols;
    const int col = threadIdx.x % cols, rl = threadIdx.x / cols;
    const int r0 = blockIdx.x * slab, r1 = min(r0 + slab, rows);
    float4 s = make_float4(0.f, 0.f, 0.f, 0.f);
    if (rl < lanes) {
#pragma unroll 4
        for (int r = r0 + rl; r < r1; r += lanes) {
            const float4 v = reinterpret_cast<const float4*>(in + (int64_t)r * W)[col];
            s.x += v.x; s.y += v.y; s.z += v.z; s.w += v.w;
        }
    }
    red[threadIdx.x] = s;
    __syncthreads();
    if (rl == 0) {
        for (int l = 1; l < lanes; ++l) { const float4 u = red[l * cols + col]; s.x += u.x; s.y += u.y; s.z += u.z; s.w += u.w; }
        reinterpret_cast<float4*>(out + (int64_t)blockIdx.x * W)[col] = s;
    }
}

__device__ __forceinline__ bool col_pair_sums(const float* __restrict__ partial, int nblocks, int C, double (&r0)[4][4], double (&r1)[4][4],
                                              double& s0, double& s1) {
    const int lc = threadIdx.x & 3, lr = threadIdx.x >> 2;
    const int c = blockIdx.x * 4 + lc;
    s0 = 0.0; s1 = 0.0;
    if (c < C) {
        double t0[8] = {0, 0, 0, 0, 0, 0, 0, 0}, t1[8] = {0, 0, 0, 0, 0, 0, 0, 0};
        for (int b = lr; b < nblocks; b += 64 * 8) {
            float v0[8], v1[8];
#pragma unroll
            for (int u = 0; u < 8; ++u) {
                const int row = b + 64 * u;
                const int64_t o = (int64_t)(row < nblocks ? row : 0) * 2 * C + c;
                v0[u] = partial[o];
                v1[u] = partial[o + C];
// ... 104 lines not shown
        float4 o;
        o.x = (v.x - mu.x) * is.x * g.x + b.x; o.y = (v.y - mu.y) * is.y * g.y + b.y;
        o.z = (v.z - mu.z) * is.z * g.z + b.z; o.w = (v.w - mu.w) * is.w * g.w + b.w;
        if (res) {
            const float4 r = ld4(res, i);
            o.x += r.x; o.y += r.y; o.z += r.z; o.w += r.w;
        }
        if (mask) mask[i] = (uint8_t)((o.x > 0.f ? 1 : 0) | (o.y > 0.f ? 2 : 0) | (o.z > 0.f ? 4 : 0) | (o.w > 0.f ? 8 : 0));
        if (relu) { o.x = fmaxf(o.x, 0.f); o.y = fmaxf(o.y, 0.f); o.z = fmaxf(o.z, 0.f); o.w = fmaxf(o.w, 0.f); }
        st4(y, i, o);
    }
}

__global__ __launch_bounds__(256) void k_bn_fold(const float* gamma, const float* beta, const float* rm, const float* rv, float eps,
                                                  int C, float* scale, float* shift) {
    const int c = blockIdx.x * 256 + threadIdx.x;
    if (c >= C) return;
    const float s = gamma[c] / sqrtf(rv[c] + eps);
    scale[c] = s;
    shift[c] = beta[c] - rm[c] * s;
}

template <typename T>
__global__ __launch_bounds__(256) void k_bn_bwd_apply(const T* __restrict__ dy, const T* __restrict__ x, const T* __restrict__ y,
                                                       int relu, int64_t n4, int C, const float* __restrict__ mean,
                                                       const float* __restrict__ invstd, const float* __restrict__ gamma,
                                                       const float* __restrict__ beta, const float* __restrict__ mg,
                                                       const float* __restrict__ mgx, T* __restrict__ dx, T* __restrict__ g_out) {
    const int64_t stride = (int64_t)gridDim.x * 256;
    const int cols = C >> 2;
    const bool fixed = stride % cols == 0;
    const int col0 = (int)(((int64_t)blockIdx.x * 256 + threadIdx.x) % cols);
    float4 mu = reinterpret_cast<const float4*>(mean)[col0], is = reinterpret_cast<const float4*>(invstd)[col0];
    float4 ga = reinterpret_cast<const float4*>(gamma)[col0];
    float4 be = relu == 2 ? reinterpret_cast<const float4*>(beta)[col0] : make_float4(0.f, 0.f, 0.f, 0.f);
    float4 a = reinterpret_cast<const float4*>(mg)[col0], b = reinterpret_cast<const float4*>(mgx)[col0];
    for (int64_t i = (int64_t)blockIdx.x * 256 + threadIdx.x; i < n4; i += stride) {
        float4 g = ld4(dy, i);
        const float4 xv = ld4(x, i);
        if (!fixed) {
            const int col = (int)(i % cols);
            mu = reinterpret_cast<const float4*>(mean)[col]; is = reinterpret_cast<const float4*>(invstd)[col];
            ga = reinterpret_cast<const float4*>(gamma)[col];
            if (relu == 2) be = reinterpret_cast<const float4*>(beta)[col];
            a = reinterpret_cast<const float4*>(mg)[col]; b = reinterpret_cast<const float4*>(mgx)[col];
        }
        if (relu == 1) {
            const float4 yy = ld4(y, i);
            g.x = yy.x > 0.f ? g.x : 0.f; g.y = yy.y > 0.f ? g.y : 0.f; g.z = yy.z > 0.f ? g.z : 0.f; g.w = yy.w > 0.f ? g.w : 0.f;
        } else if (relu == 3) {
            const uint8_t mb = reinterpret_cast<const uint8_t*>(y)[i];
            g.x = (mb & 1) ? g.x : 0.f; g.y = (mb & 2) ? g.y : 0.f; g.z = (mb & 4) ? g.z : 0.f; g.w = (mb & 8) ? g.w : 0.f;
        } else if (relu == 2) {
            g.x = ((xv.x - mu.x) * is.x * ga.x + be.x) > 0.f ? g.x : 0.f; g.y = ((xv.y - mu.y) * is.y * ga.y + be.y) > 0.f ? g.y : 0.f;
            g.z = ((xv.z - mu.z) * is.z * ga.z + be.z) > 0.f ? g.z : 0.f; g.w = ((xv.w - mu.w) * is.w * ga.w + be.w) > 0.f ? g.w : 0.f;
        }
        float4 o;
        o.x = ga.x * is.x * (g.x - a.x - (xv.x - mu.x) * is.x * b.x);
        o.y = ga.y * is.y * (g.y - a.y - (xv.y - mu.y) * is.y * b.y);
        o.z = ga.z * is.z * (g.z - a.z - (xv.z - mu.z) * is.z * b.z);
        o.w = ga.w * is.w * (g.w - a.w - (xv.w - mu.w) * is.w * b.w);
        st4(dx, i, o);
        if (g_out) st4(g_out, i, g);
    }
}

__global__ __launch_bounds__(256) void k_maxpool_fwd(const float* __restrict__ x, float* __restrict__ y, uint8_t* __restrict__ idx, int B,
                                                      int Hi, int Wi, int Ho, int Wo, int C) {
    const int cols = C >> 2;
    const int64_t n4 = (int64_t)B * Ho * Wo * cols;
    const int64_t i = (int64_t)blockIdx.x * 256 + threadIdx.x;
    if (i >= n4) return;
    const int col = (int)(i % cols);
    int64_t t = i / cols;
    const int ox = (int)(t % Wo); t /= Wo;
    const int oy = (int)(t % Ho);
    const int b = (int)(t / Ho);
    float4 m = make_float4(-INFINITY, -INFINITY, -INFINITY, -INFINITY);
    uchar4 w = make_uchar4(0, 0, 0, 0);
#pragma unroll
    for (int r = 0; r < 3; ++r) {
#pragma unroll
        for (int s = 0; s < 3; ++s) {
            const int iy = oy * 2 - 1 + r, ix = ox * 2 - 1 + s;
            if (iy < 0 || iy >= Hi || ix < 0 || ix >= Wi) continue;
            const float4 v = reinterpret_cast<const float4*>(x + (((int64_t)b * Hi + iy) * Wi + ix) * C)[col];
            const uint8_t tap = (uint8_t)(r * 3 + s);
            if (v.x > m.x) { m.x = v.x; w.x = tap; }
            if (v.y > m.y) { m.y = v.y; w.y = tap; }
            if (v.z > m.z) { m.z = v.z; w.z = tap; }
            if (v.w > m.w) { m.w = v.w; w.w = tap; }
        }
    }
    reinterpret_cast<float4*>(y)[i] = m;
    reinterpret_cast<uchar4*>(idx)[i] = w;
}

__global__ __launch_bounds__(256) void k_maxpool_bwd(const float* __restrict__ dy, const uint8_t* __restrict__ idx, float* __restrict__ dx,
                                                      int B, int Hi, int Wi, int Ho, int Wo, int C) {
    const int cols = C >> 2;
    const int64_t n4 = (int64_t)B * Hi * Wi * cols;
    const int64_t i = (int64_t)blockIdx.x * 256 + threadIdx.x;
    if (i >= n4) return;
    const int col = (int)(i % cols);
    int64_t t = i / cols;
    const int ix = (int)(t % Wi); t /= Wi;
    const int iy = (int)(t % Hi);
    const int b = (int)(t / Hi);
    float4 acc = make_float4(0.f, 0.f, 0.f, 0.f);
    for (int oy = (iy + 1) / 2 - ((iy + 1) % 2 == 0 ? 1 : 0); oy <= (iy + 1) / 2; ++oy) {
        if (oy < 0 || oy >= Ho) continue;
        const int r = iy - (oy * 2 - 1);
        if (r < 0 || r > 2) continue;
        for (int ox = (ix + 1) / 2 - ((ix + 1) % 2 == 0 ? 1 : 0); ox <= (ix + 1) / 2; ++ox) {
            if (ox < 0 || ox >= Wo) continue;
            const int s = ix - (ox * 2 - 1);
// ... 425 lines not shown
    int stage = 0;
    for (; tile < ntiles; tile += nwaves) {
        const int nst = stage == 0 ? HF_NST - 1 : stage - 1;
        HF_ISSUE(tile + (HF_NST - 1) * nwaves, nst)
        wait_vmcnt<8 * (HF_NST - 1)>();
        const uint32_t a0 = t_base + (uint32_t)stage * 8192u + (uint32_t)row * 512u;
        f32x4 a[8];
#pragma unroll
        for (int j = 0; j < 8; ++j) a[j] = lds_read128_async<0>(a0 + (uint32_t)(((4 * j + kq) ^ row) << 4));
        SD_LDS_WAIT4(0, a[0], a[1], a[2], a[3]);
        SD_LDS_WAIT4(0, a[4], a[5], a[6], a[7]);
        f32x4 acc0 = {0.f, 0.f, 0.f, 0.f}, acc1 = {0.f, 0.f, 0.f, 0.f};
#pragma unroll
        for (int j = 0; j < 8; j += 2)
#pragma unroll
            for (int t = 0; t < 4; ++t) {
                acc0 = __builtin_amdgcn_mfma_f32_16x16x4f32(a[j][t], bw[j][t], acc0, 0, 0, 0);
                acc1 = __builtin_amdgcn_mfma_f32_16x16x4f32(a[j + 1][t], bw[j + 1][t], acc1, 0, 0, 0);
            }
        if (row < Co) {
            const uint32_t m0 = (uint32_t)tile * 16u;
            const uint32_t b = m0 / (uint32_t)HW, pix = m0 - b * (uint32_t)HW;
            const f32x4 o = {acc0[0] + acc1[0] + bv, acc0[1] + acc1[1] + bv, acc0[2] + acc1[2] + bv, acc0[3] + acc1[3] + bv};
            *reinterpret_cast<f32x4*>(y + ((int64_t)b * Co + row) * HW + pix + 4 * kq) = o;
        }
        stage = stage + 1 == HF_NST ? 0 : stage + 1;
    }
    wait_vmcnt<0>();
#undef HF_ISSUE
}

constexpr int HEAD_WG_PIX = 1024;
template <typename T>
__global__ __launch_bounds__(256) void k_head_dgrad(const float* __restrict__ dy, const float* __restrict__ w, T* __restrict__ dx,
                                                     int64_t M, int HW, int C, int Co) {
    __shared__ float gs[HEAD_NARROW_MAX_CO][64];
    extern __shared__ __attribute__((aligned(16))) float lds[];
    float* ws = lds;
    const int64_t m0 = (int64_t)blockIdx.x * 64;
    for (int i = threadIdx.x; i < Co * 64; i += 256) {
        const int co = i >> 6, px = i & 63;
        const int64_t m = m0 + px;
        float v = 0.f;
        if (m < M) { const int64_t b = m / HW, pix = m - b * HW; v = dy[(b * Co + co) * HW + pix]; }
        gs[co][px] = v;
    }
    for (int i = threadIdx.x; i < Co * C; i += 256) ws[i] = w[i];
    __syncthreads();
    const int c4 = C >> 2;
    for (int i = threadIdx.x; i < 64 * c4; i += 256) {
        const int row = i / c4, col = i - row * c4;
        const int64_t m = m0 + row;
        if (m >= M) continue;
        float4 o = make_float4(0.f, 0.f, 0.f, 0.f);
        for (int co = 0; co < Co; ++co) {
            const float g = gs[co][row];
            const float4 ww = *reinterpret_cast<const float4*>(ws + co * C + col * 4);
            o.x += g * ww.x; o.y += g * ww.y; o.z += g * ww.z; o.w += g * ww.w;
        }
        if constexpr (sizeof(T) == 2) {
            uint2 pk;
            pk.x = (uint32_t)f32_to_bf16(o.x) | ((uint32_t)f32_to_bf16(o.y) << 16);
            pk.y = (uint32_t)f32_to_bf16(o.z) | ((uint32_t)f32_to_bf16(o.w) << 16);
            reinterpret_cast<uint2*>(dx + m * C)[col] = pk;
        } else {
            reinterpret_cast<float4*>(dx + m * C)[col] = o;
        }
    }
}

template <int CO>
__global__ __launch_bounds__(256) void k_head_wgrad_bf16(const float* __restrict__ dy, const uint16_t* __restrict__ x, float* __restrict__ partial,
                                                          int64_t M, int HW, int C, int Co) {
    __shared__ float gs[CO][64];
    __shared__ float comb[4][CO * 128];
    const int64_t mb = (int64_t)blockIdx.x * HEAD_WG_PIX;
    const int CG = C >> 3, PL = 256 / CG;
    const int cg = threadIdx.x % CG, pl = threadIdx.x / CG;
    float acc[CO][8];
#pragma unroll
    for (int j = 0; j < CO; ++j)
#pragma unroll
        for (int k = 0; k < 8; ++k) acc[j][k] = 0.f;
    float bsum = 0.f;
    for (int64_t m0 = mb; m0 < min(mb + HEAD_WG_PIX, M); m0 += 64) {
        __syncthreads();
        for (int i = threadIdx.x; i < Co * 64; i += 256) {
            const int co = i >> 6, px = i & 63;
            const int64_t m = m0 + px;
            float v = 0.f;
            if (m < M) { const int64_t b = m / HW, pix = m - b * HW; v = dy[(b * Co + co) * HW + pix]; }
            gs[co][px] = v;
        }
        __syncthreads();
        for (int p0 = 0; p0 < 64; p0 += 4 * PL) {
            uint4 xv[4];
#pragma unroll
            for (int u = 0; u < 4; ++u) {
                const int px = p0 + u * PL + pl;
                const int64_t m = m0 + px;
                xv[u] = reinterpret_cast<const uint4*>(x + (px < 64 && m < M ? m : mb) * C)[cg];
            }
#pragma unroll
            for (int u = 0; u < 4; ++u) {
                const int px = p0 + u * PL + pl;
                if (px >= 64) continue;
                const float f[8] = {__uint_as_float(xv[u].x << 16), __uint_as_float(xv[u].x & 0xffff0000u), __uint_as_float(xv[u].y << 16),
                                    __uint_as_float(xv[u].y & 0xffff0000u), __uint_as_float(xv[u].z << 16), __uint_as_float(xv[u].z & 0xffff0000u),
                                    __uint_as_float(xv[u].w << 16), __uint_as_float(xv[u].w & 0xffff0000u)};
#pragma unroll
                for (int j = 0; j < CO; ++j) {
                    if (j < Co) {
// ... 793 lines not shown
    partial = fold_partials(partial, rows, C, scratch, st);
    SD_LAUNCH_CHECK();
    bn_stats_finish(partial, rows, M, C, 0.f, 0.f, nullptr, nullptr, nullptr, nullptr, sums, st);
    SD_LAUNCH_CHECK();
    return 0;
}

int sd_bn_stats_from_sums(const double* sums, int C, float eps, float momentum, float* running_mean, float* running_var, float* mean,
                          float* invstd, sd_stream_t stream) {
    if (int e = check_mc("sd_bn_stats_from_sums", 1, C)) return e;
    SD_REQUIRE(sums && mean && invstd && (running_mean != nullptr) == (running_var != nullptr), SD_ERR_INVALID,
               "sd_bn_stats_from_sums: null pointer (running_mean and running_var are both given or both null)");
    SD_REQUIRE(aligned8(sums), SD_ERR_ALIGN, "sd_bn_stats_from_sums: the fp64 sums must be 8-byte aligned");
    hipLaunchKernelGGL(k_bn_stats_from_sums, dim3(cdiv(C, 256)), dim3(256), 0, (hipStream_t)stream, sums, C, eps, momentum, mean, invstd,
                       running_mean, running_var);
    SD_LAUNCH_CHECK();
    return 0;
}

int sd_bn_apply(const float* x, float* y, int64_t M, int C, const float* mean, const float* invstd, const float* gamma, const float* beta,
                const float* residual, int relu, uint8_t* relu_mask_out, sd_stream_t stream) {
    if (int e = check_mc("sd_bn_apply", M, C)) return e;
    SD_REQUIRE(x && y && mean && invstd && gamma && beta, SD_ERR_INVALID, "sd_bn_apply: null pointer");
    const int64_t n4 = M * C / 4;
    hipLaunchKernelGGL(k_bn_apply<float>, dim3(ew_grid(n4)), dim3(256), 0, (hipStream_t)stream, x, y, n4, C, mean, invstd, gamma, beta, residual, relu,
                       relu_mask_out);
    SD_LAUNCH_CHECK();
    return 0;
}

int sd_bn_fold(const float* gamma, const float* beta, const float* running_mean, const float* running_var, float eps, int C, float* scale,
               float* shift, sd_stream_t stream) {
    SD_REQUIRE(gamma && beta && running_mean && running_var && scale && shift && C > 0, SD_ERR_INVALID, "sd_bn_fold: bad arguments");
    hipLaunchKernelGGL(k_bn_fold, dim3(cdiv(C, 256)), dim3(256), 0, (hipStream_t)stream, gamma, beta, running_mean, running_var, eps, C, scale, shift);
    SD_LAUNCH_CHECK();
    return 0;
}

int sd_bn_bwd(const float* dy, const float* x, const float* y, int relu, int64_t M, int C, const float* mean, const float* invstd,
              const float* gamma, const float* beta, float* dx, float* g_out, float* dgamma, float* dbeta, int accumulate, void* workspace,
              size_t workspace_bytes, sd_stream_t stream) {
    SD_REQUIRE(dx, SD_ERR_INVALID, "sd_bn_bwd: null pointer");
    if (int e = bn_bwd_reduce_any<float>("sd_bn_bwd", dy, x, y, relu, M, C, mean, invstd, gamma, beta, dgamma, dbeta, accumulate, nullptr, false,
                                         workspace, workspace_bytes, (hipStream_t)stream)) return e;
    const int nb = cdiv(M, red_rows(M));
    const float* mg = (const float*)workspace + (size_t)nb * 2 * C;
    const int64_t n4 = M * C / 4;
    hipLaunchKernelGGL(k_bn_bwd_apply<float>, dim3(ew_grid(n4)), dim3(256), 0, (hipStream_t)stream, dy, x, y, relu, n4, C, mean, invstd, gamma, beta,
                       mg, mg + C, dx, g_out);
    SD_LAUNCH_CHECK();
    return 0;
}

int sd_bn_bwd_reduce(const float* dy, const float* x, const float* y, int relu, int64_t M, int C, const float* mean, const float* invstd,
                     const float* gamma, const float* beta, float* dgamma, float* dbeta, int accumulate, double* sums, void* workspace,
                     size_t workspace_bytes, sd_stream_t stream) {
    SD_REQUIRE(sums, SD_ERR_INVALID, "sd_bn_bwd_reduce: null pointer");
    return bn_bwd_reduce_any<float>("sd_bn_bwd_reduce", dy, x, y, relu, M, C, mean, invstd, gamma, beta, dgamma, dbeta, accumulate, sums, false,
                                    workspace, workspace_bytes, (hipStream_t)stream);
}

int sd_bn_bwd_finalize(const float* partial, int rows, int64_t M, int C, float* dgamma, float* dbeta, int accumulate, float* means_out,
                       float* scratch, sd_stream_t stream) {
    if (int e = check_mc("sd_bn_bwd_finalize", M, C)) return e;
    SD_REQUIRE(partial && dgamma && dbeta && means_out && rows > 0, SD_ERR_INVALID, "sd_bn_bwd_finalize: bad arguments");
    hipStream_t st = (hipStream_t)stream;
    const float* fin = fold_partials(partial, rows, C, scratch, st);
    SD_LAUNCH_CHECK();
    bn_bwd_finish(fin, rows, M, C, dgamma, dbeta, accumulate, means_out, means_out + C, nullptr, st);
    SD_LAUNCH_CHECK();
    return 0;
}

int sd_bn_bwd_sums(const float* partial, int rows, int64_t M, int C, float* dgamma, float* dbeta, int accumulate, double* sums, float* scratch,
                   sd_stream_t stream) {
    if (int e = check_mc("sd_bn_bwd_sums", M, C)) return e;
    SD_REQUIRE(partial && dgamma && dbeta && sums && rows > 0, SD_ERR_INVALID, "sd_bn_bwd_sums: bad arguments (null pointer or rows <= 0)");
    SD_REQUIRE(aligned8(sums), SD_ERR_ALIGN, "sd_bn_bwd_sums: the fp64 sums must be 8-byte aligned");
    hipStream_t st = (hipStream_t)stream;
    const float* fin = fold_partials(partial, rows, C, scratch, st);
    SD_LAUNCH_CHECK();
    bn_bwd_finish(fin, rows, M, C, dgamma, dbeta, accumulate, nullptr, nullptr, sums, st);
    SD_LAUNCH_CHECK();
    return 0;
}

int sd_bn_bwd_means_from_sums(const double* sums, int C, float* means_out, sd_stream_t stream) {
    if (int e = check_mc("sd_bn_bwd_means_from_sums", 1, C)) return e;
    SD_REQUIRE(sums && means_out, SD_ERR_INVALID, "sd_bn_bwd_means_from_sums: null pointer");
    SD_REQUIRE(aligned8(sums), SD_ERR_ALIGN, "sd_bn_bwd_means_from_sums: the fp64 sums must be 8-byte aligned");
    hipLaunchKernelGGL(k_bn_bwd_means_from_sums, dim3(cdiv(C, 256)), dim3(256), 0, (hipStream_t)stream, sums, C, means_out);
    SD_LAUNCH_CHECK();
    return 0;
}

int sd_bn_bwd_apply(const float* dy, const float* x, const float* y, int relu, int64_t M, int C, const float* mean, const float* invstd,
                    const float* gamma, const float* beta, const float* means, float* dx, float* g_out, sd_stream_t stream) {
    if (int e = check_mc("sd_bn_bwd_apply", M, C)) return e;
    SD_REQUIRE(relu >= 0 && relu <= 3, SD_ERR_INVALID, "sd_bn_bwd_apply: relu must be 0 (none), 1 (mask from y), 2 (mask recomputed from x) or 3 (mask bytes)");
    SD_REQUIRE(dy && x && mean && invstd && gamma && means && dx && ((relu != 1 && relu != 3) || y) && (relu != 2 || beta), SD_ERR_INVALID,
               "sd_bn_bwd_apply: null pointer");
    const int64_t n4 = M * C / 4;
    hipLaunchKernelGGL(k_bn_bwd_apply<float>, dim3(ew_grid(n4)), dim3(256), 0, (hipStream_t)stream, dy, x, y, relu, n4, C, mean, invstd, gamma, beta,
                       means, means + C, dx, g_out);
    SD_LAUNCH_CHECK();
    return 0;
// ... 294 lines not shown
    const int64_t n8 = (int64_t)B * Ho * Wo * C / 8;
    hipLaunchKernelGGL(k_maxpool_fwd_bf16, dim3(cdiv(n8, 256)), dim3(256), 0, (hipStream_t)stream, (const uint16_t*)x, (uint16_t*)y, B, Hi, Wi, Ho, Wo, C);
    SD_LAUNCH_CHECK();
    return 0;
}

int sd_head_fwd_bf16(const void* x, const float* w, const float* bias, float* y, int B, int HW, int C, int Co, sd_stream_t stream) {
    SD_REQUIRE(x && w && bias && y && B > 0 && HW > 0, SD_ERR_INVALID, "sd_head_fwd_bf16: bad arguments");
    if (Co > HEAD_NARROW_MAX_CO) return head_wide_fwd_bf16(x, w, bias, y, B, HW, C, Co, (hipStream_t)stream);
    SD_REQUIRE(C % 8 == 0 && C <= 512 && Co > 0 && Co <= HEAD_NARROW_MAX_CO, SD_ERR_INVALID, "sd_head_fwd_bf16: needs C %% 8 == 0, C <= 512, Co <= %d", HEAD_NARROW_MAX_CO);
    const int64_t M = (int64_t)B * HW;
    if (C == 128 && HW % 4 == 0 && aligned16(x) && aligned16(y)) {
        const int ntiles = (int)cdiv(M, 64), blocks = std::max(1, std::min(cdiv(ntiles, 4), 1024));
        if (Co <= 16) hipLaunchKernelGGL(k_head_fwd_bf16_c128<false>, dim3(blocks), dim3(256), 0, (hipStream_t)stream, (const uint16_t*)x, w, bias, y, M, HW, Co, ntiles);
        else hipLaunchKernelGGL(k_head_fwd_bf16_c128<true>, dim3(blocks), dim3(256), 0, (hipStream_t)stream, (const uint16_t*)x, w, bias, y, M, HW, Co, ntiles);
        SD_LAUNCH_CHECK();
        return 0;
    }
    const size_t lds = ((size_t)64 * (C + 4) + (size_t)Co * C) * sizeof(float);
    hipLaunchKernelGGL(k_head_fwd_bf16, dim3(cdiv(M, 64)), dim3(256), lds, (hipStream_t)stream, (const uint16_t*)x, w, bias, y, M, HW, C, Co);
    SD_LAUNCH_CHECK();
    return 0;
}

int sd_head_fwd(const float* x, const float* w, const float* bias, float* y, int B, int HW, int C, int Co, sd_stream_t stream) {
    SD_REQUIRE(x && w && bias && y && B > 0 && HW > 0, SD_ERR_INVALID, "sd_head_fwd: bad arguments");
    if (Co > HEAD_NARROW_MAX_CO) return head_wide_fwd(x, w, bias, y, B, HW, C, Co, (hipStream_t)stream);
    SD_REQUIRE(C % 4 == 0 && C <= 512 && Co > 0 && Co <= HEAD_NARROW_MAX_CO, SD_ERR_INVALID, "sd_head_fwd: needs C %% 4 == 0, C <= 512, Co <= %d", HEAD_NARROW_MAX_CO);
    const int64_t M = (int64_t)B * HW;
    if (C == 128 && Co <= 16 && HW % 16 == 0 && M < (1ll << 31) && aligned16(x) && aligned16(w) && aligned16(y)) {
        const int ntiles = (int)(M / 16);
        const size_t lds_b = (size_t)4 * HF_NST * 2048 * sizeof(float);
        static const hipError_t attr_once = hipFuncSetAttribute(reinterpret_cast<const void*>(&k_head_fwd_f32_c128), hipFuncAttributeMaxDynamicSharedMemorySize, (int)lds_b);
        SD_HIP(attr_once);
        hipLaunchKernelGGL(k_head_fwd_f32_c128, dim3(std::min(cdiv(ntiles, 4), 256)), dim3(256), lds_b, (hipStream_t)stream, x, w, bias, y, HW, Co, ntiles);
        SD_LAUNCH_CHECK();
        return 0;
    }
    const size_t lds = ((size_t)64 * (C + 4) + (size_t)Co * C) * sizeof(float);
    hipLaunchKernelGGL(k_head_fwd, dim3(cdiv(M, 64)), dim3(256), lds, (hipStream_t)stream, x, w, bias, y, M, HW, C, Co);
    SD_LAUNCH_CHECK();
    return 0;
}

static int head_wgrad_wave_rows(int64_t M) { return (int)std::min<int64_t>(1024, (cdiv(M, 16) + 3) / 4 * 4); }
size_t sd_head_bwd_workspace_bytes(int B, int HW, int C, int Co) {
    const int64_t M = (int64_t)B * HW;
    if (Co > HEAD_NARROW_MAX_CO) return head_wide_bwd_workspace_bytes(M, C, Co);
    return align_up((size_t)std::max<int64_t>(cdiv(M, HEAD_WG_PIX), head_wgrad_wave_rows(M)) * (Co * C + Co) * sizeof(float), 256);
}

int sd_head_bwd(const float* dy, const float* x, const float* w, float* dx, float* dw, float* dbias, int B, int HW, int C, int Co,
                int accumulate, void* workspace, size_t workspace_bytes, sd_stream_t stream) {
    SD_REQUIRE(dy && x && w && dx && dw && dbias && workspace && B > 0 && HW > 0, SD_ERR_INVALID, "sd_head_bwd: bad arguments");
    if (Co > HEAD_NARROW_MAX_CO) {
        const int64_t P = (int64_t)B * HW;
        if (int e = head_wide_check("sd_head_bwd", P, C, Co)) return e;
        SD_REQUIRE(workspace_bytes >= sd_head_bwd_workspace_bytes(B, HW, C, Co), SD_ERR_WORKSPACE, "sd_head_bwd: workspace too small");
        hipStream_t st = (hipStream_t)stream;
        int rows = 0;
        if (int e = head_wide_wgrad(dy, x, (float*)workspace, B, HW, C, Co, st, rows)) return e;
        const int n = Co * C + Co;
        hipLaunchKernelGGL(k_head_wgrad_fin, dim3(cdiv(n, 8)), dim3(256), 0, st, (const float*)workspace, rows, n, dw, dbias, Co * C, accumulate);
        SD_LAUNCH_CHECK();
        return head_wide_dgrad(dy, w, dx, B, HW, C, Co, st);
    }
    SD_REQUIRE(C % 4 == 0 && C <= 256 && (256 % C == 0) && (64 % (256 / C) == 0) && ((64 / (256 / C)) % 8 == 0) && Co > 0 && Co <= HEAD_NARROW_MAX_CO,
               SD_ERR_INVALID, "sd_head_bwd: needs C in {64, 128, 256} and Co <= %d", HEAD_NARROW_MAX_CO);
    SD_REQUIRE(workspace_bytes >= sd_head_bwd_workspace_bytes(B, HW, C, Co), SD_ERR_WORKSPACE, "sd_head_bwd: workspace too small");
    const int64_t M = (int64_t)B * HW;
    hipStream_t st = (hipStream_t)stream;
    int nb = cdiv(M, HEAD_WG_PIX);
    if (C == 128 && Co <= 16 && HW % 16 == 0 && M < (1ll << 31) && aligned16(x) && aligned16(dy)) {
        nb = head_wgrad_wave_rows(M);
        const int blocks = nb / 4;
        const size_t lds_b = (size_t)4 * HF_NST * HWG_STAGE * sizeof(float);
        static const hipError_t attr_once = hipFuncSetAttribute(reinterpret_cast<const void*>(&k_head_wgrad_f32_c128), hipFuncAttributeMaxDynamicSharedMemorySize, (int)lds_b);
        SD_HIP(attr_once);
        hipLaunchKernelGGL(k_head_wgrad_f32_c128, dim3(blocks), dim3(256), lds_b, st, dy, x, (float*)workspace, HW, Co, (int)(M / 16));
    } else {
        hipLaunchKernelGGL(k_head_wgrad, dim3(nb), dim3(256), 0, st, dy, x, (float*)workspace, M, HW, C, Co);
    }
    SD_LAUNCH_CHECK();
    const int n = Co * C + Co;
    hipLaunchKernelGGL(k_head_wgrad_fin, dim3(cdiv(n, 8)), dim3(256), 0, st, (const float*)workspace, nb, n, dw, dbias, Co * C, accumulate);
    SD_LAUNCH_CHECK();
    hipLaunchKernelGGL(k_head_dgrad<float>, dim3(cdiv(M, 64)), dim3(256), (size_t)Co * C * sizeof(float), st, dy, w, dx, M, HW, C, Co);
    SD_LAUNCH_CHECK();
    return 0;
}

int sd_head_bwd_bf16(const float* dy, const void* x_bf16, const float* w, void* dx_bf16, float* dw, float* dbias, int B, int HW, int C, int Co,
                     int accumulate, void* workspace, size_t workspace_bytes, sd_stream_t stream) {
    SD_REQUIRE(dy && x_bf16 && w && dx_bf16 && dw && dbias && workspace && B > 0 && HW > 0, SD_ERR_INVALID, "sd_head_bwd_bf16: bad arguments");
    SD_REQUIRE((C == 64 || C == 128) && Co > 0 && Co <= 8, SD_ERR_INVALID, "sd_head_bwd_bf16: needs C in {64, 128} and Co <= 8 (got %d, %d)", C, Co);
    SD_REQUIRE(aligned16(x_bf16) && aligned16(dx_bf16), SD_ERR_ALIGN, "sd_head_bwd_bf16: x and dx must be 16-byte aligned");
    SD_REQUIRE(workspace_bytes >= sd_head_bwd_workspace_bytes(B, HW, C, Co), SD_ERR_WORKSPACE, "sd_head_bwd_bf16: workspace too small");
    const int64_t M = (int64_t)B * HW;
    hipStream_t st = (hipStream_t)stream;
    hipLaunchKernelGGL(k_head_dgrad<uint16_t>, dim3(cdiv(M, 64)), dim3(256), (size_t)Co * C * sizeof(float), st, dy, w, (uint16_t*)dx_bf16, M, HW, C, Co);
    SD_LAUNCH_CHECK();
    const int nb = cdiv(M, HEAD_WG_PIX);
    hipLaunchKernelGGL(k_head_wgrad_bf16<8>, dim3(nb), dim3(256), 0, st, dy, (const uint16_t*)x_bf16, (float*)workspace, M, HW, C, Co);
    SD_LAUNCH_CHECK();
    const int n = Co * C + Co;
    hipLaunchKernelGGL(k_head_wgrad_fin, dim3(cdiv(n, 8)), dim3(256), 0, st, (const float*)workspace, nb, n, dw, dbias, Co * C, accumulate);
    SD_LAUNCH_CHECK();
    return 0;
}

int sd_adam_step(float* param, const float* grad, float* exp_avg, float* exp_avg_sq, int64_t n, int step, float lr, float beta1, float beta2,
                 float eps, float grad_scale, sd_stream_t stream) {
    SD_REQUIRE(param && grad && exp_avg && exp_avg_sq && n > 0 && n % 4 == 0 && step >= 1, SD_ERR_INVALID, "sd_adam_step: bad arguments (n %% 4 == 0, step >= 1)");
    SD_REQUIRE(aligned16(param) && aligned16(grad) && aligned16(exp_avg) && aligned16(exp_avg_sq), SD_ERR_ALIGN, "sd_adam_step: pointers must be 16-byte aligned");
    const double bc1 = 1.0 - pow((double)beta1, step), bc2 = 1.0 - pow((double)beta2, step);
    hipLaunchKernelGGL(k_adam, dim3(ew_grid(n / 4)), dim3(256), 0, (hipStream_t)stream, param, grad, exp_avg, exp_avg_sq, n / 4, lr, beta1, beta2, eps,
                       (float)bc1, (float)sqrt(bc2), grad_scale);
    SD_LAUNCH_CHECK();
    return 0;
}

static inline int sumsq_blocks(int64_t n) { return n > 0 ? (int)std::min<int64_t>(cdiv(n / 4, 256), SUMSQ_MAX_BLOCKS) : 0; }

size_t sd_grad_sumsq_workspace_bytes(int64_t n) { return (size_t)sumsq_blocks(n) * sizeof(double); }

int sd_grad_sumsq(const float* grad, int64_t n, void* workspace, size_t workspace_bytes, sd_stream_t stream) {
    SD_REQUIRE(grad && workspace && n > 0 && n % 4 == 0, SD_ERR_INVALID, "sd_grad_sumsq: bad arguments (n %% 4 == 0)");
    SD_REQUIRE(aligned16(grad) && (reinterpret_cast<uintptr_t>(workspace) & 7u) == 0, SD_ERR_ALIGN,
               "sd_grad_sumsq: grad must be 16-byte aligned, the workspace 8-byte aligned");
    SD_REQUIRE(workspace_bytes >= sd_grad_sumsq_workspace_bytes(n), SD_ERR_WORKSPACE, "sd_grad_sumsq: workspace too small");
    hipLaunchKernelGGL(k_grad_sumsq, dim3(sumsq_blocks(n)), dim3(256), 0, (hipStream_t)stream, grad, n / 4, (double*)workspace);
    SD_LAUNCH_CHECK();
    return 0;
}

int sd_optim_step(float* param, const float* grad, float* exp_avg, float* exp_avg_sq, int64_t n, int step, float lr, float beta1, float beta2,
                  float eps, float grad_scale, float weight_decay, const uint8_t* decay_mask, float max_norm, const void* partials,
                  int npartials, float* ema, float ema_decay, void* status, sd_stream_t stream) {
    SD_REQUIRE(param && grad && exp_avg && exp_avg_sq && n > 0 && n % 4 == 0 && step >= 1, SD_ERR_INVALID, "sd_optim_step: bad arguments (n %% 4 == 0, step >= 1)");
// ... 37 lines not shown
```

### structuredetector_amd/model/network.py

```python
from __future__ import annotations

import ctypes as C
import math
import warnings

import torch
import torch.nn as nn

from .. import _lib as L
from ..utils import trace as T

BN_EPS = 1e-5
BN_MOMENTUM = 0.1


class ConvParams(nn.Module):
    def __init__(self, cin, cout, k, stride=1, pad=0, bias=False):
        super().__init__()
        self.cin, self.cout, self.k, self.stride, self.pad = cin, cout, k, stride, pad
        w = torch.empty((cout, cin, k, k), memory_format=torch.channels_last)
        self.weight = nn.Parameter(w)
        self.bias = nn.Parameter(torch.zeros(cout)) if bias else None


# ... 41 lines not shown
        self.conv = ConvParams(in_channels, out_channels, 1, bias=True)


BACKBONE_FILE_GLOB = "resnet34-*.pth"


def find_backbone_weights(args=None):
    import os
    from pathlib import Path
    for given in (getattr(args, "backbone_weights", None), os.environ.get("SDNET_BACKBONE_WEIGHTS")):
        if given:
            path = Path(given).expanduser()
            if not path.is_file():
                raise L.SdError(f"backbone weights file not found: {path}")
            return path
    homes = []
    if os.environ.get("TORCH_HOME"):
        homes.append(Path(os.environ["TORCH_HOME"]))
    homes.append(Path(os.environ.get("XDG_CACHE_HOME", "~/.cache")).expanduser() / "torch")
    for home in homes:
        hits = sorted((home / "hub" / "checkpoints").glob(BACKBONE_FILE_GLOB))
        if hits:
            return hits[0]
    return None


def _layer(cin, cout, n, stride):
    return nn.Sequential(*[BasicBlock(cin if i == 0 else cout, cout, stride if i == 0 else 1) for i in range(n)])


def _desc(B, Hi, Wi, conv: ConvParams):
    d = L.ConvDesc()
    d.B, d.Hi, d.Wi, d.Cin, d.Cout, d.R, d.S, d.stride, d.pad = B, Hi, Wi, conv.cin, conv.cout, conv.k, conv.k, conv.stride, conv.pad
    d.Ho = (Hi + 2 * conv.pad - conv.k) // conv.stride + 1
    d.Wo = (Wi + 2 * conv.pad - conv.k) // conv.stride + 1
    return d


def _ptr(t):
    return 0 if t is None else t.data_ptr()


class _Engine:

    def __init__(self, net: "Network"):
        self.net = net
        self.lib = L.lib()
        self.prof = None
        self.prof_shapes = None
        self._nbt = []
        self.overlap_wgrad = False
        self._side = None
        self.fuse_bn_bwd = False
        self._wt_plan, self._wt_flat, self._wt_valid = None, {}, None
        self._head_ok = {}
        self.stem_ring = True
        self.fuse_head = True
        self.small_batch_kernel = True

    def _kname(self, d, which):
        if self.prof is None:
            return ""
        if self.prof_shapes is not None:
            self.prof_shapes.append((d.B, d.Hi, d.Wi, d.Cin, d.Cout, d.R, d.stride, d.Ho, d.Wo))
        return self.lib.sd_conv2d_kernel_name(C.byref(d), which).decode()

    def _timed(self, kind, flops, fn, phase="fwd"):
        if self.prof is None:
            return fn()
        e0, e1 = torch.cuda.Event(enable_timing=True), torch.cuda.Event(enable_timing=True)
        e0.record()
        fn()
        e1.record()
        self.prof.append((kind, flops, e0, e1, phase))

    def _ws(self, nbytes, dev):
        return L.workspace(max(int(nbytes), 256), dev)

    def _to_bf16(self, t):
        out = torch.empty(t.shape, dtype=torch.bfloat16, device=t.device)
        L.check(self.lib.sd_cast_f32_to_bf16(t.data_ptr(), out.data_ptr(), t.numel(), L.stream()), "sd_cast_f32_to_bf16")
        return out

    def _to_f32(self, t):
        out = torch.empty(t.shape, dtype=torch.float32, device=t.device)
        L.check(self.lib.sd_cast_bf16_to_f32(t.data_ptr(), out.data_ptr(), t.numel(), L.stream()), "sd_cast_bf16_to_f32")
        return out

    def refresh_bf16_weights(self):
        net = self.net
        if net.flat_params_bf16 is None:
            net.flat_params_bf16 = torch.empty(net.flat_params.numel(), dtype=torch.bfloat16, device=net.flat_params.device)
        L.check(self.lib.sd_cast_f32_to_bf16(net.flat_params.data_ptr(), net.flat_params_bf16.data_ptr(), net.flat_params.numel(), L.stream()),
                "sd_cast_f32_to_bf16")

    def _w16(self, conv):
        off, n = self.net._flat_off[id(conv.weight)]
        return self.net.flat_params_bf16[off:off + n]

    def _conv_sb(self, x, w, y, d, scale, shift, res, res_up2, relu, bf16):
        nws = self.lib.sd_conv2d_fwd_sb_workspace_bytes(C.byref(d), bf16)
        ws = self._ws(nws, x.device) if nws else None
        st = L.zero_state(self.lib.sd_conv2d_fwd_sb_state_bytes(C.byref(d), bf16), x.device) if nws else None
        L.check(self.lib.sd_conv2d_fwd_sb(x.data_ptr(), w.data_ptr(), y.data_ptr(), C.byref(d), _ptr(scale), _ptr(shift), _ptr(res), int(res_up2),
                                          int(relu), bf16, _ptr(ws), ws.numel() if nws else 0, _ptr(st), st.numel() if nws else 0, L.stream()),
                "sd_conv2d_fwd_sb")
# ... 316 lines not shown
                Hc, Wc = d1.Ho, d1.Wo
            feats.append((cur, Hc, Wc))
        (p2, H2, W2), (p3, H3, W3), (p4, H4, W4), (p5, H5, W5) = feats
        f, _ = self.conv_bf16(p5, net.up1, B, H5, W5, shift=net.up1.bias)
        hc = net.head.conv
        out = torch.empty((B, hc.cout, H2, W2), dtype=torch.float32, device=x.device)
        for fpn, (sc_t, Hs, Ws) in ((net.up2, (p4, H4, W4)), (net.up3, (p3, H3, W3)), (net.up4, (p2, H2, W2))):
            t, _ = self.conv_bf16(sc_t, fpn.lateral, B, Hs, Ws, shift=fpn.lateral.bias, res=f, res_up2=True)
            sf, hf = self.bn_fold(fpn.conv[1])
            if fpn is net.up4 and self.fuse_head and self._head_fusable(B, Hs, Ws, fpn.conv[0], hc):
                dl = _desc(B, Hs, Ws, fpn.conv[0])
                rc = lib.sd_conv2d_fwd_bf16_head(t.data_ptr(), self._w_bf16(fpn.conv[0]).data_ptr(), C.byref(dl), sf.data_ptr(), hf.data_ptr(), 1,
                                                 self._head_prepared(hc).data_ptr(), hc.cout, out.data_ptr(), L.stream())
                if rc == 0:
                    return out
                if rc > 0:
                    L.check(rc, "sd_conv2d_fwd_bf16_head")
                self._head_ok.pop((B, Hs, Ws, hc.cout), None)
            f, _ = self.conv_bf16(t, fpn.conv[0], B, Hs, Ws, scale=sf, shift=hf, relu=True)
        L.check(lib.sd_head_fwd_bf16(f.data_ptr(), hc.weight.data_ptr(), hc.bias.data_ptr(), out.data_ptr(), B, H2 * W2, hc.cin, hc.cout,
                                     L.stream()), "sd_head_fwd_bf16")
        return out

    def _transpose_all(self, amp):
        net = self.net
        if self._wt_plan is None:
            convs = [m for m in net.modules() if isinstance(m, ConvParams) and m.cin % 64 == 0 and m.cout % 64 == 0]
            rows, views, dst, blk = [], {}, 0, 0
            for m in convs:
                taps, n = m.k * m.k, m.weight.numel()
                nbx, nby = (m.cin + 31) // 32, (m.cout + 31) // 32
                rows.append([net._flat_off[id(m.weight)][0], dst, m.cout, taps, m.cin, blk, nbx, nby])
                views[id(m)] = (dst, n)
                dst += n; blk += nbx * nby * taps
            table = torch.tensor(rows, dtype=torch.int32, device=net.flat_params.device).contiguous()
            self._wt_plan = (table, len(convs), blk, views, dst)
        table, nconv, blocks, _, total = self._wt_plan
        key = "bf16" if amp else "f32"
        if key not in self._wt_flat:
            self._wt_flat[key] = torch.empty(total, dtype=torch.bfloat16 if amp else torch.float32, device=net.flat_params.device)
        L.check(self.lib.sd_conv2d_transpose_weights_batched(net.flat_params.data_ptr(), self._wt_flat[key].data_ptr(), table.data_ptr(), nconv, blocks,
                                                             int(amp), L.stream()), "sd_conv2d_transpose_weights_batched")
        self._wt_valid = key

    def _wt(self, conv, amp=False):
        if self._wt_valid == ("bf16" if amp else "f32") and id(conv) in self._wt_plan[3]:
            off, n = self._wt_plan[3][id(conv)]
            return self._wt_flat[self._wt_valid][off:off + n]
        wt = torch.empty(conv.cin * conv.k * conv.k * conv.cout, dtype=torch.bfloat16 if amp else torch.float32, device=conv.weight.device)
        transpose = self.lib.sd_conv2d_transpose_weights_bf16 if amp else self.lib.sd_conv2d_transpose_weights
        L.check(transpose(conv.weight.data_ptr(), wt.data_ptr(), conv.cout, conv.k * conv.k, conv.cin, L.stream()), "transpose_weights")
        return wt

    def _dgrad(self, dy, conv, d, res=None, bn_next=None, res_half=False, sync=None):
        amp = dy.dtype == torch.bfloat16
        dx = torch.empty((d.B, d.Hi, d.Wi, conv.cin), dtype=dy.dtype, device=dy.device)
        wt = self._wt(conv, amp)
        flops = 2.0 * d.B * d.Ho * d.Wo * conv.cout * conv.cin * conv.k * conv.k
        if amp:
            assert bn_next is None, "fuse_bn_bwd is an fp32-path experiment"
            mode = 2 if res_half else (1 if res is not None else 0)
            self._timed("bf16:" + self._kname(d, 17), flops, lambda: L.check(
                self.lib.sd_conv2d_dgrad_bf16(dy.data_ptr(), wt.data_ptr(), dx.data_ptr(), C.byref(d), _ptr(res), mode, L.stream()),
                "sd_conv2d_dgrad_bf16"), phase="dgrad")
            return dx
        if bn_next is None:
            if res_half:
                fn = lambda: L.check(self.lib.sd_conv2d_dgrad_half_res(dy.data_ptr(), wt.data_ptr(), dx.data_ptr(), C.byref(d), res.data_ptr(),
                                                                       L.stream()), "sd_conv2d_dgrad_half_res")
            else:
                fn = lambda: L.check(self.lib.sd_conv2d_dgrad(dy.data_ptr(), wt.data_ptr(), dx.data_ptr(), C.byref(d), _ptr(res), L.stream()),
                                     "sd_conv2d_dgrad")
            self._timed(self._kname(d, 1), flops, fn, phase="dgrad")
            return dx
        assert not res_half
        x, y, relu, bn, mean, invstd = bn_next
        ws = self._ws(self.lib.sd_conv2d_dgrad_bn_reduce_workspace_bytes(C.byref(d)), dy.device)
        if sync is not None:
            sums = sync.take(conv.cin)
            sync.record("sd_conv2d_dgrad_bn_reduce_sums")
            self._timed(self._kname(d, 1), flops, lambda: L.check(
                self.lib.sd_conv2d_dgrad_bn_reduce_sums(dy.data_ptr(), wt.data_ptr(), dx.data_ptr(), C.byref(d), _ptr(res), x.data_ptr(),
                                                        _ptr(y) if int(relu) in (1, 3) else 0, int(relu), mean.data_ptr(), invstd.data_ptr(),
                                                        bn.weight.data_ptr(), bn.bias.data_ptr(), self.net.grad_of(bn.weight).data_ptr(),
                                                        self.net.grad_of(bn.bias).data_ptr(), 0, sums.data_ptr(), ws.data_ptr(), ws.numel(),
                                                        L.stream()), "sd_conv2d_dgrad_bn_reduce_sums"), phase="dgrad")
            return dx, self._means_from_sums(sync, sums, conv.cin, dy.device)
        means = torch.empty(2 * conv.cin, dtype=torch.float32, device=dy.device)
        self._timed(self._kname(d, 1), flops, lambda: L.check(
            self.lib.sd_conv2d_dgrad_bn_reduce(dy.data_ptr(), wt.data_ptr(), dx.data_ptr(), C.byref(d), _ptr(res), x.data_ptr(),
                                               _ptr(y) if int(relu) in (1, 3) else 0, int(relu), mean.data_ptr(), invstd.data_ptr(),
                                               bn.weight.data_ptr(), bn.bias.data_ptr(), self.net.grad_of(bn.weight).data_ptr(),
                                               self.net.grad_of(bn.bias).data_ptr(), 0, means.data_ptr(), ws.data_ptr(), ws.numel(),
                                               L.stream()), "sd_conv2d_dgrad_bn_reduce"), phase="dgrad")
        return dx, means

    def _side_stream(self):
        if self._side is None:
            self._side = torch.cuda.Stream()
        return self._side

    def _wgrad(self, dy, x, conv, d):
        if not self.overlap_wgrad:
            return self._wgrad_now(dy, x, conv, d)
        main, side = torch.cuda.current_stream(), self._side_stream()
        ready = torch.cuda.Event()
        ready.record(main)
        with torch.cuda.stream(side):
            side.wait_event(ready)
            self._wgrad_now(dy, x, conv, d)
        dy.record_stream(side); x.record_stream(side)

    def _join_side(self):
        if self.overlap_wgrad and self._side is not None:
            torch.cuda.current_stream().wait_stream(self._side)

    def _wgrad_now(self, dy, x, conv, d):
        g = self.net.grad_of(conv.weight)
        flops = 2.0 * d.B * d.Ho * d.Wo * conv.cout * conv.cin * conv.k * conv.k
        if dy.dtype == torch.bfloat16:
            ws = self._ws(self.lib.sd_conv2d_wgrad_bf16_workspace_bytes(C.byref(d)), dy.device)
            self._timed("bf16:" + self._kname(d, 2), flops, lambda: L.check(
                self.lib.sd_conv2d_wgrad_bf16(dy.data_ptr(), x.data_ptr(), g.data_ptr(), C.byref(d), 0, ws.data_ptr(), ws.numel(), L.stream()),
                "sd_conv2d_wgrad_bf16"), phase="wgrad")
            return
        nbytes = self.lib.sd_conv2d_wgrad_workspace_bytes(C.byref(d))
        ws = self._ws(nbytes, dy.device)
        self._timed(self._kname(d, 2), flops, lambda: L.check(
# ... 12 lines not shown
        dx = torch.empty_like(x)
        g = torch.empty_like(x) if want_g else None
        if means is None and sync is not None:
            sums = sync.take(Cc)
            bf16 = x.dtype == torch.bfloat16
            sync.record("sd_bn_bwd_reduce_bf16" if bf16 else "sd_bn_bwd_reduce")
            ws = self._ws(self.lib.sd_col_reduce_workspace_bytes(Mrows, Cc), x.device)
            reduce = self.lib.sd_bn_bwd_reduce_bf16 if bf16 else self.lib.sd_bn_bwd_reduce
            L.check(reduce(dy.data_ptr(), x.data_ptr(), _ptr(y) if int(relu) in (1, 3) else 0, int(relu), Mrows, Cc, mean.data_ptr(),
                           invstd.data_ptr(), bn.weight.data_ptr(), bn.bias.data_ptr(), self.net.grad_of(bn.weight).data_ptr(),
                           self.net.grad_of(bn.bias).data_ptr(), 0, sums.data_ptr(), ws.data_ptr(), ws.numel(), L.stream()), "sd_bn_bwd_reduce")
            means = self._means_from_sums(sync, sums, Cc, x.device)
            apply = self.lib.sd_bn_bwd_apply_bf16 if bf16 else self.lib.sd_bn_bwd_apply
            L.check(apply(dy.data_ptr(), x.data_ptr(), _ptr(y) if int(relu) in (1, 3) else 0, int(relu), Mrows, Cc, mean.data_ptr(),
                          invstd.data_ptr(), bn.weight.data_ptr(), bn.bias.data_ptr(), means.data_ptr(), dx.data_ptr(), _ptr(g), L.stream()),
                    "sd_bn_bwd_apply")
            return dx, g
        if means is not None:
            L.check(self.lib.sd_bn_bwd_apply(dy.data_ptr(), x.data_ptr(), _ptr(y) if int(relu) in (1, 3) else 0, int(relu), Mrows, Cc,
                                             mean.data_ptr(), invstd.data_ptr(), bn.weight.data_ptr(), bn.bias.data_ptr(), means.data_ptr(),
                                             dx.data_ptr(), _ptr(g), L.stream()), "sd_bn_bwd_apply")
            return dx, g
        ws = self._ws(self.lib.sd_col_reduce_workspace_bytes(Mrows, Cc), x.device)
        bn_bwd = self.lib.sd_bn_bwd_bf16 if x.dtype == torch.bfloat16 else self.lib.sd_bn_bwd
        L.check(bn_bwd(dy.data_ptr(), x.data_ptr(), _ptr(y) if int(relu) in (1, 3) else 0, int(relu), Mrows, Cc, mean.data_ptr(),
                                   invstd.data_ptr(), bn.weight.data_ptr(), bn.bias.data_ptr(), dx.data_ptr(), _ptr(g),
                                   self.net.grad_of(bn.weight).data_ptr(),
                                   self.net.grad_of(bn.bias).data_ptr(), 0, ws.data_ptr(), ws.numel(), L.stream()), "sd_bn_bwd")
        return dx, g

    def backward(self, tape, dhead, on_stage=None):
        net, lib = self.net, self.lib
        B = tape["B"]
        H2, W2 = tape["hw"]
        dhead = dhead.contiguous().float()
        hc = net.head.conv
        amp = bool(tape.get("amp"))
        if amp and self.fuse_bn_bwd:
            raise L.SdError("fuse_bn_bwd is an fp32-path experiment; switch it off for mixed-precision training")
        sx = tape.get("bn_sync")
        if sx is not None:
            sx.begin("bwd")
        T.push("bwd:fpn_head")
        self._transpose_all(amp)
        ws = self._ws(lib.sd_head_bwd_workspace_bytes(B, H2 * W2, hc.cin, hc.cout), dhead.device)
        if amp and hc.cin in (64, 128) and hc.cout <= 8:
            f1 = tape["f1"]
            df = torch.empty_like(f1)
            L.check(lib.sd_head_bwd_bf16(dhead.data_ptr(), f1.data_ptr(), hc.weight.data_ptr(), df.data_ptr(), net.grad_of(hc.weight).data_ptr(),
                                         net.grad_of(hc.bias).data_ptr(), B, H2 * W2, hc.cin, hc.cout, 0, ws.data_ptr(), ws.numel(), L.stream()),
                    "sd_head_bwd_bf16")
        else:
            f1 = self._to_f32(tape["f1"]) if amp else tape["f1"]
            df = torch.empty_like(f1)
            L.check(lib.sd_head_bwd(dhead.data_ptr(), f1.data_ptr(), hc.weight.data_ptr(), df.data_ptr(), net.grad_of(hc.weight).data_ptr(),
                                    net.grad_of(hc.bias).data_ptr(), B, H2 * W2, hc.cin, hc.cout, 0, ws.data_ptr(), ws.numel(), L.stream()),
                    "sd_head_bwd")
            if amp:
                df = self._to_bf16(df)

        lateral_grad = {}
        for (fpn, sc_t, (Hs, Ws), dl, t, dc, c, mf, if_, fn) in reversed(tape["fpn"]):
            dcv, _ = self._bn_bwd(df, c, fn, 2, fpn.conv[1], mf, if_, sync=sx)
            dt = self._dgrad(dcv, fpn.conv[0], dc)
            self._wgrad(dcv, t, fpn.conv[0], dc)
            self._wgrad(dt, sc_t, fpn.lateral, dl)
            self._bias_grad(dt, fpn.lateral)
            lateral_grad[sc_t.data_ptr()] = (dt, fpn.lateral, dl)
            dfp = torch.empty((B, Hs // 2, Ws // 2, fpn.lateral.cout), dtype=dt.dtype, device=dt.device)
            up2_bwd = lib.sd_upsample2x_bwd_bf16 if amp else lib.sd_upsample2x_bwd
            L.check(up2_bwd(dt.data_ptr(), 0, dfp.data_ptr(), B, Hs // 2, Ws // 2, fpn.lateral.cout, L.stream()), "up2_bwd")
            df = dfp
        p5, H5, W5 = tape["p5"]
        d5 = _desc(B, H5, W5, net.up1)
        self._wgrad(df, p5, net.up1, d5)
        self._bias_grad(df, net.up1)
        blocks = tape["blocks"]

        def bn2_of(i):
            if i < 0 or not self.fuse_bn_bwd:
                return None
            b = blocks[i]
            return (b[9], b[17], 3, b[0].bn2, b[10], b[11])

        last = len(blocks) - 1
        has_lateral = blocks[last][12].data_ptr() in lateral_grad
        nxt = None if has_lateral else bn2_of(last)
        r = self._dgrad(df, net.up1, d5, bn_next=nxt, sync=sx)
        dcur, mcur = r if nxt is not None else (r, None)
        T.pop()
        if on_stage:
            self._join_side()
            on_stage("fpn_head")

        first_of = {id(net.down4[0]): "down4", id(net.down3[0]): "down3", id(net.down2[0]): "down2"}
        T.push("bwd:down4")
        for bi in range(last, -1, -1):
            (blk, xin, (Hc, Wc), d1, c1, a1, m1, i1, d2, c2, m2, i2, out, dd, cd, md, idd, msk) = blocks[bi]
            extra = lateral_grad.pop(out.data_ptr(), None)
            if extra is not None:
                nxt = bn2_of(bi)
                r = self._dgrad(extra[0], extra[1], extra[2], res=dcur, bn_next=nxt, sync=sx)
                dcur, mcur = r if nxt is not None else (r, None)
            dc2, g = self._bn_bwd(dcur, c2, msk, 3, blk.bn2, m2, i2, want_g=True, means=mcur, sync=sx)
            nxt = (c1, None, 2, blk.bn1, m1, i1) if self.fuse_bn_bwd else None
            r = self._dgrad(dc2, blk.conv2, d2, bn_next=nxt, sync=sx)
            da1, ma1 = r if nxt is not None else (r, None)
            self._wgrad(dc2, a1, blk.conv2, d2)
            dc1, _ = self._bn_bwd(da1, c1, a1, 2, blk.bn1, m1, i1, means=ma1, sync=sx)
            half = False
            if blk.downsample is not None:
                dcd, _ = self._bn_bwd(g, cd, None, False, blk.downsample[1], md, idd, sync=sx)
                ds = blk.downsample[0]
                half = ds.k == 1 and ds.stride == 2 and ds.pad == 0 and Hc % 2 == 0 and Wc % 2 == 0 and not self.fuse_bn_bwd
                if half:
                    dsm = L.ConvDesc()
                    dsm.B, dsm.Hi, dsm.Wi, dsm.Cin, dsm.Cout, dsm.R, dsm.S, dsm.stride, dsm.pad = B, dd.Ho, dd.Wo, ds.cin, ds.cout, 1, 1, 1, 0
                    dsm.Ho, dsm.Wo = dd.Ho, dd.Wo
                    skip = self._dgrad(dcd, ds, dsm)
                else:
                    skip = self._dgrad(dcd, ds, dd)
                self._wgrad(dcd, xin, ds, dd)
            else:
                skip = g
            prev_lateral = bi > 0 and blocks[bi - 1][12].data_ptr() in lateral_grad
            nxt = None if (bi == 0 or prev_lateral) else bn2_of(bi - 1)
            r = self._dgrad(dc1, blk.conv1, d1, res=skip, bn_next=nxt, res_half=half, sync=sx)
            dcur, mcur = r if nxt is not None else (r, None)
            self._wgrad(dc1, xin, blk.conv1, d1)
            if id(blk) in first_of:
                T.pop()
                if on_stage:
                    self._join_side()
                    on_stage(first_of[id(blk)])
                T.push("bwd:" + {"down4": "down3", "down3": "down2", "down2": "down1_stem"}[first_of[id(blk)]])

        d0, s0, m0, i0, pidx = tape["stem"]
        bn0 = net.adpater[1]
        amp_stem = s0.dtype == torch.bfloat16
        if amp and not amp_stem:
            dcur = self._to_f32(dcur)
        ring = amp_stem and self.stem_ring and d0.Wi % 4 == 0
        ds0 = torch.empty(s0.shape, dtype=torch.bfloat16 if ring else torch.float32, device=s0.device)
        ws = self._ws(lib.sd_col_reduce_workspace_bytes(B * d0.Ho * d0.Wo, 64), s0.device)
        if sx is None:
            pool_bwd = lib.sd_maxpool_bn_relu_bwd_bf16_dx16 if ring else (lib.sd_maxpool_bn_relu_bwd_bf16 if amp_stem else lib.sd_maxpool_bn_relu_bwd)
            L.check(pool_bwd(dcur.data_ptr(), pidx.data_ptr(), s0.data_ptr(), B, d0.Ho, d0.Wo, 64, m0.data_ptr(), i0.data_ptr(),
                             bn0.weight.data_ptr(), bn0.bias.data_ptr(), ds0.data_ptr(), net.grad_of(bn0.weight).data_ptr(),
                             net.grad_of(bn0.bias).data_ptr(), 0, ws.data_ptr(), ws.numel(), L.stream()), "sd_maxpool_bn_relu_bwd")
        else:
            sums = sx.take(64)
            sx.record("sd_maxpool_bn_relu_bwd_reduce")
            pool_reduce = lib.sd_maxpool_bn_relu_bwd_reduce_bf16 if amp_stem else lib.sd_maxpool_bn_relu_bwd_reduce
            L.check(pool_reduce(dcur.data_ptr(), pidx.data_ptr(), s0.data_ptr(), B, d0.Ho, d0.Wo, 64, m0.data_ptr(), i0.data_ptr(),
                                bn0.weight.data_ptr(), bn0.bias.data_ptr(), net.grad_of(bn0.weight).data_ptr(), net.grad_of(bn0.bias).data_ptr(), 0,
                                sums.data_ptr(), ws.data_ptr(), ws.numel(), L.stream()), "sd_maxpool_bn_relu_bwd_reduce")
            means = self._means_from_sums(sx, sums, 64, s0.device)
            pool_apply = lib.sd_maxpool_bn_relu_bwd_apply_bf16_dx16 if ring else (lib.sd_maxpool_bn_relu_bwd_apply_bf16 if amp_stem
                                                                                  else lib.sd_maxpool_bn_relu_bwd_apply)
            L.check(pool_apply(dcur.data_ptr(), pidx.data_ptr(), s0.data_ptr(), B, d0.Ho, d0.Wo, 64, m0.data_ptr(), i0.data_ptr(),
                               bn0.weight.data_ptr(), bn0.bias.data_ptr(), means.data_ptr(), ds0.data_ptr(), L.stream()), "sd_maxpool_bn_relu_bwd_apply")
        stem = net.adpater[0]
        ws = self._ws(lib.sd_conv2d_stem_wgrad_workspace_bytes(C.byref(d0)), ds0.device)
        stem_wgrad = lib.sd_conv2d_stem_wgrad_bf16 if ring else (lib.sd_conv2d_stem_wgrad_bf16mm if amp else lib.sd_conv2d_stem_wgrad)
        L.check(stem_wgrad(ds0.data_ptr(), tape["x"].data_ptr(), net.grad_of(stem.weight).data_ptr(), C.byref(d0), 0,
                           ws.data_ptr(), ws.numel(), L.stream()), "sd_conv2d_stem_wgrad")
        self._join_side()
        self._wt_valid = None
        T.pop()
        if on_stage:
            on_stage("down1_stem")


class _NetFn(torch.autograd.Function):

    @staticmethod
    def forward(ctx, net, x, *params):
        tape = {}
        out = net._engine.forward(x, True, tape)
        ctx.net, ctx.tape = net, tape
# ... 204 lines not shown
```

Baseline: 878.5.

## Recompute gradient sources in consumers instead of materializing head dx and masked g

Adds a BN-backward kernel that recomputes the head's input gradient on the fly from dhead and the head weights, so the FPN BN backward no longer needs a materialized df tensor. In residual blocks it stops writing the ReLU-masked gradient g. The downsample BN backward applies the mask itself, and a new masked-residual dgrad epilogue applies the ReLU mask to the skip gradient. This removes full-size activation writes and reads in the fp32 backward path, at the cost of redundant head matvec work per BN channel and extra mask loads in conv epilogues.

New measurement: 884.3, median of 6. No clear change (+0.7%).

```diff
diff --git a/include/sdnet_hip.h b/include/sdnet_hip.h
--- a/include/sdnet_hip.h
+++ b/include/sdnet_hip.h
@@ -294,6 +294,9 @@
                     const float* residual, sd_stream_t stream);
 int sd_conv2d_dgrad_half_res(const float* dy, const float* w_t, float* dx, const sd_conv_desc* d, const float* residual_half,
                              sd_stream_t stream);
+int sd_conv2d_dgrad_masked_res_supported(const sd_conv_desc* d);
+int sd_conv2d_dgrad_masked_res(const float* dy, const float* w_t, float* dx, const sd_conv_desc* d, const float* residual,
+                               const uint8_t* residual_mask, sd_stream_t stream);
 int sd_conv2d_transpose_weights(const float* w, float* w_t, int Cout, int taps, int Cin, sd_stream_t stream);
 int sd_conv2d_transpose_weights_batched(const float* w_base, void* w_t_base, const int* table, int nconv, int total_blocks, int out_bf16,
                                         sd_stream_t stream);
@@ -320,6 +323,9 @@
 int sd_bn_bwd(const float* dy, const float* x, const float* y, int relu, int64_t M, int C, const float* mean,
               const float* invstd, const float* gamma, const float* beta, float* dx, float* g_out, float* dgamma,
               float* dbeta, int accumulate, void* workspace, size_t workspace_bytes, sd_stream_t stream);
+int sd_bn_bwd_head(const float* dhead_nchw, const float* head_w, int Co, int HW, const float* x, int relu, int64_t M, int C,
+                   const float* mean, const float* invstd, const float* gamma, const float* beta, float* dx, float* dgamma,
+                   float* dbeta, int accumulate, void* workspace, size_t workspace_bytes, sd_stream_t stream);
 int sd_col_sum(const float* x, int64_t M, int C, float* out, int accumulate, void* workspace,
                size_t workspace_bytes, sd_stream_t stream);
 
diff --git a/structuredetector_amd/_lib.py b/structuredetector_amd/_lib.py
--- a/structuredetector_amd/_lib.py
+++ b/structuredetector_amd/_lib.py
@@ -140,6 +140,9 @@
     "sd_stem_bn_relu_maxpool_fwd_bf16": (c_int, [c_vp, c_vp, c_vp, c_vp, c_vp, c_vp, c_vp]),
     "sd_head_fwd_bf16": (c_int, [c_vp, c_vp, c_vp, c_vp, c_int, c_int, c_int, c_int, c_vp]),
     "sd_conv2d_dgrad": (c_int, [c_vp, c_vp, c_vp, C.POINTER(ConvDesc), c_vp, c_vp]),
+    "sd_conv2d_dgrad_masked_res_supported": (c_int, [C.POINTER(ConvDesc)]),
+    "sd_conv2d_dgrad_masked_res": (c_int, [c_vp, c_vp, c_vp, C.POINTER(ConvDesc), c_vp, c_vp, c_vp]),
+    "sd_bn_bwd_head": (c_int, [c_vp, c_vp, c_int, c_int, c_vp, c_int, c_i64, c_int, c_vp, c_vp, c_vp, c_vp, c_vp, c_vp, c_vp, c_int, c_vp, c_size, c_vp]),
     "sd_conv2d_transpose_weights": (c_int, [c_vp, c_vp, c_int, c_int, c_int, c_vp]),
     "sd_conv2d_transpose_weights_batched": (c_int, [c_vp, c_vp, c_vp, c_int, c_int, c_int, c_vp]),
     "sd_conv2d_wgrad_workspace_bytes": (c_size, [C.POINTER(ConvDesc)]),
diff --git a/structuredetector_amd/csrc/sd_conv.hip b/structuredetector_amd/csrc/sd_conv.hip
--- a/structuredetector_amd/csrc/sd_conv.hip
+++ b/structuredetector_amd/csrc/sd_conv.hip
@@ -86,6 +86,7 @@
     const float* head_b;
     float* head_y;
     int head_co;
+    const uint8_t* res_mask;
 };
 
 __device__ __attribute__((aligned(128))) float g_zero_line[64];
@@ -572,7 +573,7 @@
     }
 }
 
-template <int BN, int WM, int WN, int MT, int NTW, bool FWD, bool BF16 = false, bool VEC = false, typename RowMap, typename ResMap>
+template <int BN, int WM, int WN, int MT, int NTW, bool FWD, bool BF16 = false, bool VEC = false, bool MASKRES = false, typename RowMap, typename ResMap>
 __device__ __forceinline__ void tile_epilogue(const ConvArgs& p, f32x16 (&acc)[MT][NTW], RowMap row_to_m, ResMap row_to_res, int tid, int wave, int fr,
                                               int fh, int wm0, int wn0, int n0, int tile_m, float* T0 = nullptr, float* T1 = nullptr) {
     const bool fwd_stat = FWD && p.stat && !p.bn_x;
@@ -629,7 +630,7 @@
                     T0[r * 64 + ni * 32 + fr] = v0;
                     if (two) T1[r * 64 + ni * 32 + fr] = v1;
                 }
-            auto out_row = [&](int it, uint2 r16) {
+            auto out_row = [&](int it, uint2 r16, auto masked) {
                 const int rl = it * 4 + (lane >> 4);
                 const int trow = wm0 + h * rpp + rl;
                 const int m = row_to_m(trow);
@@ -643,7 +644,14 @@
                             v.x += bf2f((uint16_t)(r16.x & 0xffff)); v.y += bf2f((uint16_t)(r16.x >> 16));
                             v.z += bf2f((uint16_t)(r16.y & 0xffff)); v.w += bf2f((uint16_t)(r16.y >> 16));
                         } else {
-                            const float4 r = *reinterpret_cast<const float4*>(reinterpret_cast<const float*>(p.res) + rm * p.Nn + n);
+                            float4 r = *reinterpret_cast<const float4*>(reinterpret_cast<const float*>(p.res) + rm * p.Nn + n);
+                            if constexpr (decltype(masked)::value) {
+                                const int mb = p.res_mask[(rm * p.Nn + n) >> 2];
+                                r.x = __uint_as_float(__float_as_uint(r.x) & (uint32_t)__builtin_amdgcn_sbfe(mb, 0, 1));
+                                r.y = __uint_as_float(__float_as_uint(r.y) & (uint32_t)__builtin_amdgcn_sbfe(mb, 1, 1));
+                                r.z = __uint_as_float(__float_as_uint(r.z) & (uint32_t)__builtin_amdgcn_sbfe(mb, 2, 1));
+                                r.w = __uint_as_float(__float_as_uint(r.w) & (uint32_t)__builtin_amdgcn_sbfe(mb, 3, 1));
+                            }
                             v.x += r.x; v.y += r.y; v.z += r.z; v.w += r.w;
                         }
                     }
@@ -662,13 +670,18 @@
             if constexpr (BF16) {
 #pragma unroll
                 for (int it = 0; it < 16; ++it)
-                    if (it * 4 < rpp) out_row(it, rr[it]);
+                    if (it * 4 < rpp) out_row(it, rr[it], std::false_type{});
             } else {
+                auto rows = [&](auto masked) {
 #pragma unroll 4
-                for (int it = 0; it < 16; ++it) {
-                    if (it * 4 >= rpp) break;
-                    out_row(it, make_uint2(0u, 0u));
-                }
+                    for (int it = 0; it < 16; ++it) {
+                        if (it * 4 >= rpp) break;
+                        out_row(it, make_uint2(0u, 0u), masked);
+                    }
+                };
+                if constexpr (MASKRES) {
+                    if (p.res_mask) rows(std::true_type{}); else rows(std::false_type{});
+                } else rows(std::false_type{});
             }
         }
         if (bwd_red) {
@@ -1168,7 +1181,7 @@
 #undef PT_PB
     __syncthreads();
     float* T0 = BN == 128 ? (wave < 3 ? Pt + wave * 4096 : Bs) : Pt + wave * 2048;
-    tile_epilogue<BN, WM, WN, MT, NTW, true, BF16, true>(
+    tile_epilogue<BN, WM, WN, MT, NTW, true, BF16, true, !BF16>(
         p, acc, [&](int row) { return m0 + row; },
         [&](int, int m) {
             const int ox = m % p.Wo, t = m / p.Wo, oy = t % p.Ho, b = t / p.Ho;
@@ -1900,6 +1913,7 @@
     const float* scale;
     const float* shift;
     const float* res;
+    const uint8_t* res_mask;
     float* stat;
     int relu, flip;
     int B, H, W, segs, rows, units_per_col, nunits;
@@ -1979,6 +1993,11 @@
             if (p.res) {
 #pragma unroll
                 for (int e = 0; e < 16; ++e) resv[e] = p.res[orow + ((e & 3) + 8 * (e >> 2)) * 64];
+            }
+            uint32_t resm[16];
+            if (p.res_mask) {
+#pragma unroll
+                for (int e = 0; e < 16; ++e) resm[e] = p.res_mask[(orow >> 2) + ((e & 3) + 8 * (e >> 2)) * 16];
             }
             const bool more = y + 3 <= y1;
             float* const ddst = reinterpret_cast<float*>(ring + ((y + 3 - y0 + 1) % RF_NR) * RF_ROW_BYTES);
@@ -2029,6 +2048,11 @@
             PP_T(r2_)
             wait_vmcnt<0>();
             PP_T(r3_)
+            if (p.res_mask) {
+#pragma unroll
+                for (int e = 0; e < 16; ++e)
+                    resv[e] = __uint_as_float(__float_as_uint(resv[e]) & (uint32_t)__builtin_amdgcn_sbfe((int)resm[e], fr & 3, 1));
+            }
 #pragma unroll
             for (int e = 0; e < 16; ++e) {
                 float v = acc[e] * sc + sh;
@@ -4526,7 +4550,7 @@
     r.nunits = cols * r.units_per_col;
     if (r.nunits < g_rowsf32_min_units || (g_rowsf32_min_units > 1 && r.rows < 16)) return false;
     r.x = (const float*)a.x; r.w = (const float*)a.w; r.y = (float*)a.y; r.scale = a.scale; r.shift = a.shift;
-    r.res = (const float*)a.res; r.stat = a.stat; r.relu = a.relu; r.flip = a.rsign < 0;
+    r.res = (const float*)a.res; r.res_mask = a.res ? a.res_mask : nullptr; r.stat = a.stat; r.relu = a.relu; r.flip = a.rsign < 0;
     return true;
 }
 
@@ -5186,6 +5210,30 @@
     return launch_igemm(a, false, (hipStream_t)stream);
 }
 
+static bool plan_takes_masked_res(const ConvPlan& p) {
+    return !p.bf16 && (p.family == CONV_PATCH || p.family == CONV_PATCH_ROLL || p.family == CONV_ROWS_F32);
+}
+
+int sd_conv2d_dgrad_masked_res_supported(const sd_conv_desc* d) {
+    if (!d || d->B <= 0 || d->Ho <= 0 || d->Wo <= 0 || d->Cout <= 0 || d->Cout % 32 || d->Cin <= 0 || d->Cin % 64) return 0;
+    return plan_takes_masked_res(plan_query(d, 1, false, false)) ? 1 : 0;
+}
+
+int sd_conv2d_dgrad_masked_res(const float* dy, const float* w_t, float* dx, const sd_conv_desc* d, const float* residual,
+                               const uint8_t* residual_mask, sd_stream_t stream) {
+    if (int e = check_conv("sd_conv2d_dgrad_masked_res", d)) return e;
+    SD_REQUIRE(dy && w_t && dx && residual && residual_mask, SD_ERR_INVALID, "sd_conv2d_dgrad_masked_res: null pointer");
+    SD_REQUIRE(d->Cout % 32 == 0 && d->Cin % 64 == 0, SD_ERR_INVALID, "sd_conv2d_dgrad_masked_res: needs Cout %% 32 == 0 and Cin %% 64 == 0");
+    SD_REQUIRE(aligned16(dy) && aligned16(w_t) && aligned16(dx) && aligned16(residual), SD_ERR_ALIGN,
+               "sd_conv2d_dgrad_masked_res: pointers must be 16-byte aligned");
+    ConvArgs a = conv_args(d, 1, false);
+    a.x = dy; a.w = w_t; a.y = dx; a.res = residual; a.res_mask = residual_mask;
+    const ConvPlan p = plan_conv(a, false);
+    SD_REQUIRE(plan_takes_masked_res(p), SD_ERR_INVALID,
+               "sd_conv2d_dgrad_masked_res: this geometry's kernel has no masked-residual epilogue (ask sd_conv2d_dgrad_masked_res_supported)");
+    return launch_plan(p, (hipStream_t)stream);
+}
+
 int sd_conv2d_transpose_weights(const float* w, float* w_t, int Cout, int taps, int Cin, sd_stream_t stream) {
     SD_REQUIRE(w && w_t && Cout > 0 && taps > 0 && Cin > 0, SD_ERR_INVALID, "sd_conv2d_transpose_weights: bad arguments");
     hipLaunchKernelGGL(k_transpose_w<float>, dim3(cdiv(Cin, 32), cdiv(Cout, 32), taps), dim3(256), 0, (hipStream_t)stream, w, w_t, Cout, taps, Cin);
diff --git a/structuredetector_amd/csrc/sd_nn.hip b/structuredetector_amd/csrc/sd_nn.hip
--- a/structuredetector_amd/csrc/sd_nn.hip
+++ b/structuredetector_amd/csrc/sd_nn.hip
@@ -5,6 +5,34 @@
 namespace sd {
 
 constexpr int RED_ROWS_PER_BLOCK = 256;
+
+__device__ __forceinline__ void bn_mask_from_x4(float4& g, const float4& xv, const float4& mu, const float4& is, const float4& ga, const float4& be) {
+    g.x = ((xv.x - mu.x) * is.x * ga.x + be.x) > 0.f ? g.x : 0.f; g.y = ((xv.y - mu.y) * is.y * ga.y + be.y) > 0.f ? g.y : 0.f;
+    g.z = ((xv.z - mu.z) * is.z * ga.z + be.z) > 0.f ? g.z : 0.f; g.w = ((xv.w - mu.w) * is.w * ga.w + be.w) > 0.f ? g.w : 0.f;
+}
+__device__ __forceinline__ void bn_bwd_sums_add4(float4& s0, float4& s1, const float4& g, const float4& xv, const float4& mu, const float4& is) {
+    s0.x += g.x; s0.y += g.y; s0.z += g.z; s0.w += g.w;
+    s1.x += g.x * ((xv.x - mu.x) * is.x); s1.y += g.y * ((xv.y - mu.y) * is.y);
+    s1.z += g.z * ((xv.z - mu.z) * is.z); s1.w += g.w * ((xv.w - mu.w) * is.w);
+}
+__device__ __forceinline__ float4 bn_bwd_dx4(const float4& g, const float4& xv, const float4& mu, const float4& is, const float4& ga, const float4& a,
+                                             const float4& b) {
+    float4 o;
+    o.x = ga.x * is.x * (g.x - a.x - (xv.x - mu.x) * is.x * b.x);
+    o.y = ga.y * is.y * (g.y - a.y - (xv.y - mu.y) * is.y * b.y);
+    o.z = ga.z * is.z * (g.z - a.z - (xv.z - mu.z) * is.z * b.z);
+    o.w = ga.w * is.w * (g.w - a.w - (xv.w - mu.w) * is.w * b.w);
+    return o;
+}
+__device__ __forceinline__ float4 head_dgrad4(const float* g, int gstride, const float* w4, int C, int Co) {
+    float4 o = make_float4(0.f, 0.f, 0.f, 0.f);
+    for (int co = 0; co < Co; ++co) {
+        const float gv = g[co * gstride];
+        const float4 ww = *reinterpret_cast<const float4*>(w4 + co * C);
+        o.x += gv * ww.x; o.y += gv * ww.y; o.z += gv * ww.z; o.w += gv * ww.w;
+    }
+    return o;
+}
 
 template <int MODE, typename T = float>
 __global__ __launch_bounds__(256) void k_col_reduce(const T* __restrict__ a, const T* __restrict__ b, const T* __restrict__ y,
@@ -41,16 +69,63 @@
                     g.x = yy.x > 0.f ? g.x : 0.f; g.y = yy.y > 0.f ? g.y : 0.f;
                     g.z = yy.z > 0.f ? g.z : 0.f; g.w = yy.w > 0.f ? g.w : 0.f;
                 } else if (relu == 2) {
-                    g.x = ((xv.x - mu.x) * is.x * ga.x + be.x) > 0.f ? g.x : 0.f; g.y = ((xv.y - mu.y) * is.y * ga.y + be.y) > 0.f ? g.y : 0.f;
-                    g.z = ((xv.z - mu.z) * is.z * ga.z + be.z) > 0.f ? g.z : 0.f; g.w = ((xv.w - mu.w) * is.w * ga.w + be.w) > 0.f ? g.w : 0.f;
+                    bn_mask_from_x4(g, xv, mu, is, ga, be);
                 } else if (relu == 3) {
                     const uint8_t mb = reinterpret_cast<const uint8_t*>(y)[r * cols + col];
                     g.x = (mb & 1) ? g.x : 0.f; g.y = (mb & 2) ? g.y : 0.f; g.z = (mb & 4) ? g.z : 0.f; g.w = (mb & 8) ? g.w : 0.f;
                 }
-                s0.x += g.x; s0.y += g.y; s0.z += g.z; s0.w += g.w;
-                s1.x += g.x * ((xv.x - mu.x) * is.x); s1.y += g.y * ((xv.y - mu.y) * is.y);
-                s1.z += g.z * ((xv.z - mu.z) * is.z); s1.w += g.w * ((xv.w - mu.w) * is.w);
+                bn_bwd_sums_add4(s0, s1, g, xv, mu, is);
             }
+        }
+    }
+    red[0][threadIdx.x] = s0;
+    red[1][threadIdx.x] = s1;
+    __syncthreads();
+    if (rl == 0) {
+        for (int l = 1; l < lanes; ++l) {
+            const float4 u = red[0][l * cols + col], w = red[1][l * cols + col];
+            s0.x += u.x; s0.y += u.y; s0.z += u.z; s0.w += u.w;
+            s1.x += w.x; s1.y += w.y; s1.z += w.z; s1.w += w.w;
+        }
+        float* dst = partial + (int64_t)blockIdx.x * 2 * C;
+        reinterpret_cast<float4*>(dst)[col] = s0;
+        reinterpret_cast<float4*>(dst + C)[col] = s1;
+    }
+}
+
+__global__ __launch_bounds__(256) void k_col_reduce_head(const float* __restrict__ dhead, const float* __restrict__ hw, int Co, int HW,
+                                                         const float* __restrict__ b, const float* __restrict__ mean, const float* __restrict__ invstd,
+                                                         const float* __restrict__ gamma, const float* __restrict__ beta, int relu,
+                                                         int64_t M, int C, float* __restrict__ partial, int rpb) {
+    __shared__ float4 red[2][256];
+    extern __shared__ __attribute__((aligned(16))) float lds[];
+    float* ws = lds;
+    float* gs = lds + Co * C;
+    const int cols = C >> 2;
+    const int lanes = 256 / cols;
+    const int col = threadIdx.x % cols, rl = threadIdx.x / cols;
+    const int64_t r0 = (int64_t)blockIdx.x * rpb;
+    const int64_t r1 = min(r0 + rpb, M);
+    const int nr = (int)(r1 - r0);
+    for (int i = threadIdx.x; i < Co * nr; i += 256) {
+        const int co = i / nr, rr = i - co * nr;
+        const int64_t m = r0 + rr, bb = m / HW, pix = m - bb * HW;
+        gs[co * rpb + rr] = dhead[(bb * Co + co) * HW + pix];
+    }
+    for (int i = threadIdx.x; i < Co * C; i += 256) ws[i] = hw[i];
+    __syncthreads();
+    float4 s0 = make_float4(0.f, 0.f, 0.f, 0.f), s1 = s0;
+    float4 mu = s0, is = s0, ga = s0, be = s0;
+    if (rl < lanes) {
+        mu = reinterpret_cast<const float4*>(mean)[col];
+        is = reinterpret_cast<const float4*>(invstd)[col];
+        if (relu == 2) { ga = reinterpret_cast<const float4*>(gamma)[col]; be = reinterpret_cast<const float4*>(beta)[col]; }
+#pragma unroll 4
+        for (int64_t r = r0 + rl; r < r1; r += lanes) {
+            float4 g = head_dgrad4(gs + (int)(r - r0), rpb, ws + col * 4, C, Co);
+            const float4 xv = ld4(b, r * cols + col);
+            if (relu == 2) bn_mask_from_x4(g, xv, mu, is, ga, be);
+            bn_bwd_sums_add4(s0, s1, g, xv, mu, is);
         }
     }
     red[0][threadIdx.x] = s0;
@@ -261,16 +336,45 @@
             const uint8_t mb = reinterpret_cast<const uint8_t*>(y)[i];
             g.x = (mb & 1) ? g.x : 0.f; g.y = (mb & 2) ? g.y : 0.f; g.z = (mb & 4) ? g.z : 0.f; g.w = (mb & 8) ? g.w : 0.f;
         } else if (relu == 2) {
-            g.x = ((xv.x - mu.x) * is.x * ga.x + be.x) > 0.f ? g.x : 0.f; g.y = ((xv.y - mu.y) * is.y * ga.y + be.y) > 0.f ? g.y : 0.f;
-            g.z = ((xv.z - mu.z) * is.z * ga.z + be.z) > 0.f ? g.z : 0.f; g.w = ((xv.w - mu.w) * is.w * ga.w + be.w) > 0.f ? g.w : 0.f;
-        }
-        float4 o;
-        o.x = ga.x * is.x * (g.x - a.x - (xv.x - mu.x) * is.x * b.x);
-        o.y = ga.y * is.y * (g.y - a.y - (xv.y - mu.y) * is.y * b.y);
-        o.z = ga.z * is.z * (g.z - a.z - (xv.z - mu.z) * is.z * b.z);
-        o.w = ga.w * is.w * (g.w - a.w - (xv.w - mu.w) * is.w * b.w);
-        st4(dx, i, o);
+            bn_mask_from_x4(g, xv, mu, is, ga, be);
+        }
+        st4(dx, i, bn_bwd_dx4(g, xv, mu, is, ga, a, b));
         if (g_out) st4(g_out, i, g);
+    }
+}
+
+__global__ __launch_bounds__(256) void k_bn_bwd_apply_head(const float* __restrict__ dhead, const float* __restrict__ hw, int Co, int HW,
+                                                           const float* __restrict__ x, int relu, int64_t M, int C, const float* __restrict__ mean,
+                                                           const float* __restrict__ invstd, const float* __restrict__ gamma,
+                                                           const float* __restrict__ beta, const float* __restrict__ mg,
+                                                           const float* __restrict__ mgx, float* __restrict__ dx) {
+    __shared__ float gs[HEAD_NARROW_MAX_CO][64];
+    extern __shared__ __attribute__((aligned(16))) float lds[];
+    float* ws = lds;
+    const int64_t m0 = (int64_t)blockIdx.x * 64;
+    for (int i = threadIdx.x; i < Co * 64; i += 256) {
+        const int co = i >> 6, px = i & 63;
+        const int64_t m = m0 + px;
+        float v = 0.f;
+        if (m < M) { const int64_t bb = m / HW, pix = m - bb * HW; v = dhead[(bb * Co + co) * HW + pix]; }
+        gs[co][px] = v;
+    }
+    for (int i = threadIdx.x; i < Co * C; i += 256) ws[i] = hw[i];
+    __syncthreads();
+    const int c4 = C >> 2;
+    const int col = threadIdx.x % c4;
+    const float4 mu = reinterpret_cast<const float4*>(mean)[col], is = reinterpret_cast<const float4*>(invstd)[col];
+    const float4 ga = reinterpret_cast<const float4*>(gamma)[col];
+    const float4 be = relu == 2 ? reinterpret_cast<const float4*>(beta)[col] : make_float4(0.f, 0.f, 0.f, 0.f);
+    const float4 a = reinterpret_cast<const float4*>(mg)[col], b = reinterpret_cast<const float4*>(mgx)[col];
+    for (int i = threadIdx.x; i < 64 * c4; i += 256) {
+        const int row = i / c4;
+        const int64_t m = m0 + row;
+        if (m >= M) break;
+        float4 g = head_dgrad4(&gs[0][row], 64, ws + col * 4, C, Co);
+        const float4 xv = ld4(x, m * c4 + col);
+        if (relu == 2) bn_mask_from_x4(g, xv, mu, is, ga, be);
+        st4(dx, m * c4 + col, bn_bwd_dx4(g, xv, mu, is, ga, a, b));
     }
 }
 
@@ -802,12 +906,7 @@
         const int row = i / c4, col = i - row * c4;
         const int64_t m = m0 + row;
         if (m >= M) continue;
-        float4 o = make_float4(0.f, 0.f, 0.f, 0.f);
-        for (int co = 0; co < Co; ++co) {
-            const float g = gs[co][row];
-            const float4 ww = *reinterpret_cast<const float4*>(ws + co * C + col * 4);
-            o.x += g * ww.x; o.y += g * ww.y; o.z += g * ww.z; o.w += g * ww.w;
-        }
+        const float4 o = head_dgrad4(&gs[0][row], 64, ws + col * 4, C, Co);
         if constexpr (sizeof(T) == 2) {
             uint2 pk;
             pk.x = (uint32_t)f32_to_bf16(o.x) | ((uint32_t)f32_to_bf16(o.y) << 16);
@@ -1707,6 +1806,36 @@
     return 0;
 }
 
+int sd_bn_bwd_head(const float* dhead, const float* head_w, int Co, int HW, const float* x, int relu, int64_t M, int C, const float* mean,
+                   const float* invstd, const float* gamma, const float* beta, float* dx, float* dgamma, float* dbeta, int accumulate,
+                   void* workspace, size_t workspace_bytes, sd_stream_t stream) {
+    if (int e = check_mc("sd_bn_bwd_head", M, C)) return e;
+    SD_REQUIRE(Co > 0 && Co <= HEAD_NARROW_MAX_CO, SD_ERR_INVALID, "sd_bn_bwd_head: narrow heads only (Co <= %d, got %d)", HEAD_NARROW_MAX_CO, Co);
+    SD_REQUIRE(HW > 0 && M % HW == 0, SD_ERR_INVALID, "sd_bn_bwd_head: M must be a multiple of HW");
+    SD_REQUIRE(relu == 0 || relu == 2, SD_ERR_INVALID, "sd_bn_bwd_head: relu must be 0 (none) or 2 (mask recomputed from x)");
+    SD_REQUIRE(dhead && head_w && x && mean && invstd && gamma && dx && dgamma && dbeta && workspace && (relu != 2 || beta), SD_ERR_INVALID,
+               "sd_bn_bwd_head: null pointer");
+    SD_REQUIRE(workspace_bytes >= sd_col_reduce_workspace_bytes(M, C), SD_ERR_WORKSPACE, "sd_bn_bwd_head: workspace too small");
+    const int rpb = red_rows(M), nb = cdiv(M, rpb);
+    const size_t lds_reduce = ((size_t)Co * C + (size_t)Co * rpb) * sizeof(float), lds_apply = (size_t)Co * C * sizeof(float);
+    SD_REQUIRE(lds_reduce <= 48 * 1024, SD_ERR_INVALID, "sd_bn_bwd_head: Co * (C + %d) floats must fit 48 KB of LDS (Co=%d, C=%d)", rpb, Co, C);
+    hipStream_t st = (hipStream_t)stream;
+    float* partial = (float*)workspace;
+    float* mg = partial + (size_t)nb * 2 * C;
+    float* mgx = mg + C;
+    hipLaunchKernelGGL(k_col_reduce_head, dim3(nb), dim3(256), lds_reduce, st, dhead, head_w, Co, HW, x, mean, invstd, gamma, beta, relu, M, C,
+                       partial, rpb);
+    SD_LAUNCH_CHECK();
+    int rows = nb;
+    const float* fin = fold_partials(partial, rows, C, mgx + C, st);
+    bn_bwd_finish(fin, rows, M, C, dgamma, dbeta, accumulate, mg, mgx, nullptr, st);
+    SD_LAUNCH_CHECK();
+    hipLaunchKernelGGL(k_bn_bwd_apply_head, dim3(cdiv(M, 64)), dim3(256), lds_apply, st, dhead, head_w, Co, HW, x, relu, M, C, mean, invstd, gamma,
+                       beta, mg, mgx, dx);
+    SD_LAUNCH_CHECK();
+    return 0;
+}
+
 int sd_bn_bwd_reduce(const float* dy, const float* x, const float* y, int relu, int64_t M, int C, const float* mean, const float* invstd,
                      const float* gamma, const float* beta, float* dgamma, float* dbeta, int accumulate, double* sums, void* workspace,
                      size_t workspace_bytes, sd_stream_t stream) {
@@ -2107,7 +2236,7 @@
 
 int sd_head_bwd(const float* dy, const float* x, const float* w, float* dx, float* dw, float* dbias, int B, int HW, int C, int Co,
                 int accumulate, void* workspace, size_t workspace_bytes, sd_stream_t stream) {
-    SD_REQUIRE(dy && x && w && dx && dw && dbias && workspace && B > 0 && HW > 0, SD_ERR_INVALID, "sd_head_bwd: bad arguments");
+    SD_REQUIRE(dy && x && w && (dx || Co <= HEAD_NARROW_MAX_CO) && dw && dbias && workspace && B > 0 && HW > 0, SD_ERR_INVALID, "sd_head_bwd: bad arguments");
     if (Co > HEAD_NARROW_MAX_CO) {
         const int64_t P = (int64_t)B * HW;
         if (int e = head_wide_check("sd_head_bwd", P, C, Co)) return e;
@@ -2140,6 +2269,7 @@
     const int n = Co * C + Co;
     hipLaunchKernelGGL(k_head_wgrad_fin, dim3(cdiv(n, 8)), dim3(256), 0, st, (const float*)workspace, nb, n, dw, dbias, Co * C, accumulate);
     SD_LAUNCH_CHECK();
+    if (!dx) return 0;
     hipLaunchKernelGGL(k_head_dgrad<float>, dim3(cdiv(M, 64)), dim3(256), (size_t)Co * C * sizeof(float), st, dy, w, dx, M, HW, C, Co);
     SD_LAUNCH_CHECK();
     return 0;
diff --git a/structuredetector_amd/model/network.py b/structuredetector_amd/model/network.py
--- a/structuredetector_amd/model/network.py
+++ b/structuredetector_amd/model/network.py
@@ -117,6 +117,7 @@
         self.overlap_wgrad = False
         self._side = None
         self.fuse_bn_bwd = False
+        self.grad_sources = True
         self._wt_plan, self._wt_flat, self._wt_valid = None, {}, None
         self._head_ok = {}
         self.stem_ring = True
@@ -539,13 +540,17 @@
         L.check(transpose(conv.weight.data_ptr(), wt.data_ptr(), conv.cout, conv.k * conv.k, conv.cin, L.stream()), "transpose_weights")
         return wt
 
-    def _dgrad(self, dy, conv, d, res=None, bn_next=None, res_half=False, sync=None):
+    def _masked_res_ok(self, d):
+        return bool(self.lib.sd_conv2d_dgrad_masked_res_supported(C.byref(d)))
+
+    def _dgrad(self, dy, conv, d, res=None, bn_next=None, res_half=False, sync=None, res_mask=None):
         amp = dy.dtype == torch.bfloat16
         dx = torch.empty((d.B, d.Hi, d.Wi, conv.cin), dtype=dy.dtype, device=dy.device)
         wt = self._wt(conv, amp)
         flops = 2.0 * d.B * d.Ho * d.Wo * conv.cout * conv.cin * conv.k * conv.k
         if amp:
             assert bn_next is None, "fuse_bn_bwd is an fp32-path experiment"
+            assert res_mask is None, "the masked residual is an fp32 epilogue"
             mode = 2 if res_half else (1 if res is not None else 0)
             self._timed("bf16:" + self._kname(d, 17), flops, lambda: L.check(
                 self.lib.sd_conv2d_dgrad_bf16(dy.data_ptr(), wt.data_ptr(), dx.data_ptr(), C.byref(d), _ptr(res), mode, L.stream()),
@@ -555,12 +560,15 @@
             if res_half:
                 fn = lambda: L.check(self.lib.sd_conv2d_dgrad_half_res(dy.data_ptr(), wt.data_ptr(), dx.data_ptr(), C.byref(d), res.data_ptr(),
                                                                        L.stream()), "sd_conv2d_dgrad_half_res")
+            elif res_mask is not None:
+                fn = lambda: L.check(self.lib.sd_conv2d_dgrad_masked_res(dy.data_ptr(), wt.data_ptr(), dx.data_ptr(), C.byref(d), res.data_ptr(),
+                                                                         res_mask.data_ptr(), L.stream()), "sd_conv2d_dgrad_masked_res")
             else:
                 fn = lambda: L.check(self.lib.sd_conv2d_dgrad(dy.data_ptr(), wt.data_ptr(), dx.data_ptr(), C.byref(d), _ptr(res), L.stream()),
                                      "sd_conv2d_dgrad")
             self._timed(self._kname(d, 1), flops, fn, phase="dgrad")
             return dx
-        assert not res_half
+        assert not res_half and res_mask is None
         x, y, relu, bn, mean, invstd = bn_next
         ws = self._ws(self.lib.sd_conv2d_dgrad_bn_reduce_workspace_bytes(C.byref(d)), dy.device)
         if sync is not None:
@@ -679,8 +687,10 @@
                     "sd_head_bwd_bf16")
         else:
             f1 = self._to_f32(tape["f1"]) if amp else tape["f1"]
-            df = torch.empty_like(f1)
-            L.check(lib.sd_head_bwd(dhead.data_ptr(), f1.data_ptr(), hc.weight.data_ptr(), df.data_ptr(), net.grad_of(hc.weight).data_ptr(),
+            head_src = (self.grad_sources and not amp and sx is None and not self.fuse_bn_bwd and hc.cout <= 32 and hc.cin in (64, 128, 256)
+                        and hc.cout * (hc.cin + 256) * 4 <= 48 * 1024 and len(tape["fpn"]) > 0 and tape["fpn"][-1][6].shape[-1] == hc.cin)
+            df = None if head_src else torch.empty_like(f1)
+            L.check(lib.sd_head_bwd(dhead.data_ptr(), f1.data_ptr(), hc.weight.data_ptr(), _ptr(df), net.grad_of(hc.weight).data_ptr(),
                                     net.grad_of(hc.bias).data_ptr(), B, H2 * W2, hc.cin, hc.cout, 0, ws.data_ptr(), ws.numel(), L.stream()),
                     "sd_head_bwd")
             if amp:
@@ -688,7 +698,16 @@
 
         lateral_grad = {}
         for (fpn, sc_t, (Hs, Ws), dl, t, dc, c, mf, if_, fn) in reversed(tape["fpn"]):
-            dcv, _ = self._bn_bwd(df, c, fn, 2, fpn.conv[1], mf, if_, sync=sx)
+            if df is None:
+                bn = fpn.conv[1]
+                Mrows, Cc = c.numel() // c.shape[-1], c.shape[-1]
+                dcv = torch.empty_like(c)
+                ws = self._ws(lib.sd_col_reduce_workspace_bytes(Mrows, Cc), c.device)
+                L.check(lib.sd_bn_bwd_head(dhead.data_ptr(), hc.weight.data_ptr(), hc.cout, H2 * W2, c.data_ptr(), 2, Mrows, Cc, mf.data_ptr(),
+                                           if_.data_ptr(), bn.weight.data_ptr(), bn.bias.data_ptr(), dcv.data_ptr(), net.grad_of(bn.weight).data_ptr(),
+                                           net.grad_of(bn.bias).data_ptr(), 0, ws.data_ptr(), ws.numel(), L.stream()), "sd_bn_bwd_head")
+            else:
+                dcv, _ = self._bn_bwd(df, c, fn, 2, fpn.conv[1], mf, if_, sync=sx)
             dt = self._dgrad(dcv, fpn.conv[0], dc)
             self._wgrad(dcv, t, fpn.conv[0], dc)
             self._wgrad(dt, sc_t, fpn.lateral, dl)
@@ -729,7 +748,9 @@
                 nxt = bn2_of(bi)
                 r = self._dgrad(extra[0], extra[1], extra[2], res=dcur, bn_next=nxt, sync=sx)
                 dcur, mcur = r if nxt is not None else (r, None)
-            dc2, g = self._bn_bwd(dcur, c2, msk, 3, blk.bn2, m2, i2, want_g=True, means=mcur, sync=sx)
+            no_g = (self.grad_sources and not amp and sx is None and not self.fuse_bn_bwd
+                    and (blk.downsample is not None or self._masked_res_ok(d1)))
+            dc2, g = self._bn_bwd(dcur, c2, msk, 3, blk.bn2, m2, i2, want_g=not no_g, means=mcur, sync=sx)
             nxt = (c1, None, 2, blk.bn1, m1, i1) if self.fuse_bn_bwd else None
             r = self._dgrad(dc2, blk.conv2, d2, bn_next=nxt, sync=sx)
             da1, ma1 = r if nxt is not None else (r, None)
@@ -737,7 +758,10 @@
             dc1, _ = self._bn_bwd(da1, c1, a1, 2, blk.bn1, m1, i1, means=ma1, sync=sx)
             half = False
             if blk.downsample is not None:
-                dcd, _ = self._bn_bwd(g, cd, None, False, blk.downsample[1], md, idd, sync=sx)
+                if no_g:
+                    dcd, _ = self._bn_bwd(dcur, cd, msk, 3, blk.downsample[1], md, idd, sync=sx)
+                else:
+                    dcd, _ = self._bn_bwd(g, cd, None, False, blk.downsample[1], md, idd, sync=sx)
                 ds = blk.downsample[0]
                 half = ds.k == 1 and ds.stride == 2 and ds.pad == 0 and Hc % 2 == 0 and Wc % 2 == 0 and not self.fuse_bn_bwd
                 if half:
@@ -749,10 +773,11 @@
                     skip = self._dgrad(dcd, ds, dd)
                 self._wgrad(dcd, xin, ds, dd)
             else:
-                skip = g
+                skip = dcur if no_g else g
             prev_lateral = bi > 0 and blocks[bi - 1][12].data_ptr() in lateral_grad
             nxt = None if (bi == 0 or prev_lateral) else bn2_of(bi - 1)
-            r = self._dgrad(dc1, blk.conv1, d1, res=skip, bn_next=nxt, res_half=half, sync=sx)
+            r = self._dgrad(dc1, blk.conv1, d1, res=skip, bn_next=nxt, res_half=half, sync=sx,
+                            res_mask=msk if (no_g and blk.downsample is None) else None)
             dcur, mcur = r if nxt is not None else (r, None)
             self._wgrad(dc1, xin, blk.conv1, d1)
             if id(blk) in first_of:
```
